# carlosmwh1985/BspAtom

Hardware: AMD Instinct MI355X
Metric: l-channel eigensolves/sec at N_bsp=4096 fp64 (higher is better)
Workload: dtype f64; 1 GPU; Hydrogen Coulomb l=0..127, N_bsp=4096, k=9, KIND_GRID=0 rb=800 (BASELINE configs[3]); `value` = weak scaling: 128 l-channels per GPU, 128 in total; channels_total=128, eigenvector_owner_rank=0, collective_calls=0, launched_by=python

## Files before the change

bspatom_amd/csrc/capi.hip:

```cpp
#include <atomic>
#include <new>
#include "capi_internal.h"

using namespace bsp;

namespace bsp {
static std::atomic<int> g_process_device{-1};
int process_device() { return g_process_device.load(); }
int process_device_check(int device)
{
    const int cur = g_process_device.load();
    if (cur >= 0 && cur != device) {
        fprintf(stderr, "bspatom: this process already works on device %d; use one process per GPU (device %d refused)\n", cur, device);
        return BSP_ERR_UNSUPPORTED;
    }
    return BSP_OK;
}
void process_device_latch(int device) { int expect = -1; g_process_device.compare_exchange_strong(expect, device); }

int device_cus()
{
    static const int cus = [] {
        int dev = 0, v = 0;
        return (hipGetDevice(&dev) == hipSuccess && hipDeviceGetAttribute(&v, hipDeviceAttributeMultiprocessorCount, dev) == hipSuccess && v > 0) ? v : 256;
    }();
    return cus;
}

hipError_t LaunchCtx::sync()
{
    hipError_t first = hipSuccess;
    auto wait = [&](hipStream_t s) {
        const hipError_t e = s ? hipStreamSynchronize(s) : hipSuccess;
        if (first == hipSuccess) first = e;
    };
    for (hipStream_t s : cw_aux) wait(s);
    for (const Sy2sbLane &ln : lanes) { wait(ln.main); wait(ln.side); }
    return first;
}

void LaunchCtx::release()
{
    (void)sync();
    auto drop_stream = [](hipStream_t &s) { if (s) (void)hipStreamDestroy(s); s = nullptr; };
    auto drop_event = [](hipEvent_t &e) { if (e) (void)hipEventDestroy(e); e = nullptr; };
    for (hipStream_t &s : cw_aux) drop_stream(s);
    drop_event(cw_fork);
    for (hipEvent_t &e : cw_join) drop_event(e);
    for (Sy2sbLane &ln : lanes) { drop_stream(ln.main); drop_stream(ln.side); drop_event(ln.evA); drop_event(ln.evB); drop_event(ln.done); }
    drop_event(sy_fork);
    (void)hipFree(bis_tail); (void)hipFree(bis_qcnt); (void)hipFree(sb2st_chk);
    bis_tail = nullptr; bis_tail_cap = 0; bis_qcnt = nullptr; sb2st_chk = nullptr;
}
}

namespace {
struct OptName { const char *name; const char *env; int Options::*field; };
const OptName OPT_TABLE[] = {
    {"sb2st_version", "BSP_SB2ST_VERSION", &Options::sb2st_version},
    {"sb2st_ring", "BSP_SB2ST_RING", &Options::sb2st_ring},
    {"sb2st_margin", "BSP_SB2ST_MARGIN", &Options::sb2st_margin},
    {"sb2st_hyst", "BSP_SB2ST_HYST", &Options::sb2st_hyst},
    {"sb2st_lead", "BSP_SB2ST_LEAD", &Options::sb2st_lead},
    {"sb2st_check", "BSP_SB2ST_CHECK", &Options::sb2st_check},
    {"sb2st_diag", "BSP_SB2ST_DIAG", &Options::sb2st_diag},
    {"sb2st_force_abort", "BSP_SB2ST_FORCE_ABORT", &Options::sb2st_force_abort},
    {"sy2sb_groups", "BSP_SY2SB_GROUPS", &Options::sy2sb_groups},
    {"sy2sb_lookahead", "BSP_SY2SB_LOOKAHEAD", &Options::sy2sb_lookahead},
    {"sy2sb_segs", "BSP_SY2SB_SEGS", &Options::sy2sb_segs},
    {"panel_qr", "BSP_PANEL_QR", &Options::panel_qr},
    {"gemm_diag", "BSP_GEMM_DIAG", &Options::gemm_diag},
    {"bisect", "BSP_BISECT", &Options::bisect},
    {"bisect_ept", "BSP_BISECT_EPT", &Options::bisect_ept},
    {"bisect_tail", "BSP_BISECT_TAIL", &Options::bisect_tail},
    {"bisect_secant", "BSP_BISECT_SECANT", &Options::bisect_secant},
    {"bisect_pair", "BSP_BISECT_PAIR", &Options::bisect_pair},
    {"bisect_queue", "BSP_BISECT_QUEUE", &Options::bisect_queue},
    {"bisect_queue_grid", "BSP_BISECT_QUEUE_GRID", &Options::bisect_queue_grid},
    {"bisect_diag", "BSP_BISECT_DIAG", &Options::bisect_diag},
    {"no_eigvec_prefetch", "BSP_NO_EIGVEC_PREFETCH", &Options::no_eigvec_prefetch},
    {"vec_early", "BSP_VEC_EARLY", &Options::vec_early},
    {"vec_own_cu", "BSP_VEC_OWN_CU", &Options::vec_own_cu},
    {"poison_c", "BSP_POISON_C", &Options::poison_c},
    {"sb2sb_mfma", "BSP_SB2SB_MFMA", &Options::sb2sb_mfma},
    {"ktime", "BSP_KTIME", &Options::ktime},
    {"tsqr_regcap", "BSP_TSQR_REGCAP", &Options::tsqr_regcap},
    {"tsqr_max_m", "BSP_TSQR_MAX_M", &Options::tsqr_max_m},
    {"sb16_rows", "BSP_SB16_ROWS", &Options::sb16_rows},
    {"route", "BSP_ROUTE", &Options::route},
    {"cw_onediv", "BSP_CW_ONEDIV", &Options::cw_onediv},
    {"cw_items4", "BSP_CW_ITEMS4", &Options::cw_items4},
    {"cw_bcast", "BSP_CW_BCAST", &Options::cw_bcast},
    {"cw_nw", "BSP_CW_NW", &Options::cw_nw},
    {"cw_ldspad", "BSP_CW_LDSPAD", &Options::cw_ldspad},
    {"cw_ipw", "BSP_CW_IPW", &Options::cw_ipw},
    {"cw_band8", "BSP_CW_BAND8", &Options::cw_band8},
    {"cw_split", "BSP_CW_SPLIT", &Options::cw_split},
    {"cw_diag", "BSP_CW_DIAG", &Options::cw_diag},
    {"s_overlap", "BSP_S_OVERLAP", &Options::s_overlap},
    {"cw_streams", "BSP_CW_STREAMS", &Options::cw_streams},
    {"cw_chunk_min", "BSP_CW_CHUNK_MIN", &Options::cw_chunk_min},
    {"sb8_wgs", "BSP_SB8_WGS", &Options::sb8_wgs},
    {"sbr_phased", "BSP_SBR_PHASED", &Options::sbr_phased},
    {"sbr_lag", "BSP_SBR_LAG", &Options::sbr_lag},
    {"fused_probe", "BSP_FUSED_PROBE", &Options::fused_probe},
    {"dipole_stage_mb", "BSP_DIPOLE_STAGE_MB", &Options::dipole_stage_mb},
    {"resolvent_stage_mb", "BSP_RESOLVENT_STAGE_MB", &Options::resolvent_stage_mb},
    {"resolvent_slots", "BSP_RESOLVENT_SLOTS", &Options::resolvent_slots},
    {"wf_stage_mb", "BSP_WF_STAGE_MB", &Options::wf_stage_mb},
    {"tdse_stage_mb", "BSP_TDSE_STAGE_MB", &Options::tdse_stage_mb},
    {"tdse_adapt_group", "BSP_TDSE_ADAPT_GROUP", &Options::tdse_adapt_group},
    {"tdse_spline_group", "BSP_TDSE_SPLINE_GROUP", &Options::tdse_spline_group},
};
}

namespace bsp {
Options &opts()
{
    static Options o = [] {
        Options v;
        for (const OptName &t : OPT_TABLE) {
            const char *e = getenv(t.env);
            if (e) v.*(t.field) = (*e == 0) ? 1 : atoi(e);
        }
        return v;
    }();
    return o;
}

namespace {
struct KRec { int slot; hipEvent_t e0, e1; };
std::vector<KRec> g_krecs;
std::vector<hipEvent_t> g_kpool;
hipEvent_t g_kopen[KS_COUNT];
hipEvent_t kevent()
{
    hipEvent_t e = nullptr;
    if (!g_kpool.empty()) { e = g_kpool.back(); g_kpool.pop_back(); }
    else if (hipEventCreate(&e) != hipSuccess) e = nullptr;
    return e;
}
const char *const KSLOT_NAMES[KS_COUNT] = {"gemm2_kernel<128,128,MODE 1> (rank-128 update, syr2k)", "gemm2_kernel<64,128,MODE 2> (symm Y = A22 W)",
                                          "panel_qr2_kernel / panel_qr_kernel", "sy2sb chain: G, K (split-K gemm_kernel + splitk_reduce), form_T, tsmm64 (W, Z)",
                                          "sb2sb_mfma_kernel (band 64 -> 16)", "sbr_rows_kernel<8> / <16> / sb16st_kernel (one-column chase to tridiagonal)", "bisect3_kernel",
                                          "band_cholesky_kernel + std_form_kernel",
                                          "crawford_item_kernel and its set-up kernels (band route: pencil -> band 15)",
                                          "operator_band_kernel (bands of caller-given g(r), g(r) d/dr)",
                                          "tdse_stage_kernel (one Runge-Kutta stage of bspatom_tdse_propagate)"};
}
void ktime_begin(int slot, hipStream_t st)
{
    hipEvent_t e = kevent();
    g_kopen[slot] = e;
    if (e) (void)hipEventRecord(e, st);
}
void ktime_end(int slot, hipStream_t st)
{
    hipEvent_t e0 = g_kopen[slot], e1 = kevent();
    g_kopen[slot] = nullptr;
    if (!e0 || !e1) return;
    (void)hipEventRecord(e1, st);
    g_krecs.push_back({slot, e0, e1});
}
}

extern "C" int bspatom_kernel_times(double *ms, int32_t *launches, int cap)
{
    if (!ms || !launches || cap < KS_COUNT) return BSP_ERR_ARG;
    BSP_HIP(hipDeviceSynchronize());
    for (int i = 0; i < cap; ++i) { ms[i] = 0.0; launches[i] = 0; }
    for (const auto &r : g_krecs) {
        float t = 0.f;
        if (hipEventElapsedTime(&t, r.e0, r.e1) == hipSuccess) { ms[r.slot] += t; launches[r.slot] += 1; }
        g_kpool.push_back(r.e0); g_kpool.push_back(r.e1);
    }
    g_krecs.clear();
    return KS_COUNT;
}

extern "C" const char *bspatom_kernel_slot_name(int slot)
{
    return (slot >= 0 && slot < KS_COUNT) ? KSLOT_NAMES[slot] : nullptr;
}

extern "C" int bspatom_set_option(const char *name, int value)
{
    if (!name) return BSP_ERR_ARG;
    for (const OptName &t : OPT_TABLE)
        if (!strcmp(name, t.name)) { opts().*(t.field) = value; return BSP_OK; }
    return BSP_ERR_ARG;
}

extern "C" int bspatom_get_option(const char *name, int *value)
{
    if (!name || !value) return BSP_ERR_ARG;
    for (const OptName &t : OPT_TABLE)
        if (!strcmp(name, t.name)) { *value = opts().*(t.field); return BSP_OK; }
    return BSP_ERR_ARG;
}

extern "C" void bspatom_input_defaults(bspatom_input *in) { input_defaults(in); }

extern "C" int bspatom_device_count(void)
{
    int n = 0;
    if (hipGetDeviceCount(&n) != hipSuccess) return 0;
    return n;
}

static int derive_checked(const bspatom_input &in, HostSetup *h)
{
    const int drc = derive(in, h);
    if (drc == -5) {
        fprintf(stderr, "bspatom: B-spline order k = %d (Gauss-Legendre points ka = %d) exceeds the limits k <= %d, ka <= %d of this build\n",
                in.k, h->ka, BSPATOM_MAX_K, BSPATOM_MAX_KA);
        return BSP_ERR_UNSUPPORTED;
    }
    return drc ? BSP_ERR_ARG : BSP_OK;
}

static void fill_sizes(const HostSetup &h, int npad, bspatom_sizes *s)
{
    s->nfun = h.nfun; s->k = h.k; s->ka = h.ka; s->nkp = h.nkp; s->nointv = h.nointv;
    s->nbc1 = h.nbc1; s->nbc2 = h.nbc2; s->lmax = h.lmax; s->nintv_exp = h.nintv_exp;
    s->nintv_lin = h.nintv_lin; s->npad = npad;
}

static void copy_grid(const HostSetup &h, double *rt, double *aind, double *xg, double *wg)
{
    if (rt) memcpy(rt, h.rt.data(), h.rt.size() * sizeof(double));
    if (aind) memcpy(aind, h.aind.data(), h.aind.size() * sizeof(double));
    if (xg) memcpy(xg, h.xg.data(), h.xg.size() * sizeof(double));
    if (wg) memcpy(wg, h.wg.data(), h.wg.size() * sizeof(double));
}

extern "C" int bspatom_host_setup(const bspatom_input *in, bspatom_sizes *s, double *rt, double *aind, double *xg,
                                  double *wg)
{
    if (!in || !s) return BSP_ERR_ARG;
    HostSetup h;
    int rc;
    if ((rc = derive_checked(*in, &h))) return rc;
    fill_sizes(h, round_up(h.nfun, 64), s);
    if (rt || aind || xg || wg) {
        build_grid(&h);
        copy_grid(h, rt, aind, xg, wg);
    }
    return BSP_OK;
}

static void free_solve_buffers(bspatom_problem *p)
{
    hipFree(p->d_SB); hipFree(p->d_HB); hipFree(p->d_UB); hipFree(p->d_rdiag); hipFree(p->d_Y);
    hipFree(p->d_C); hipFree(p->d_AB); hipFree(p->d_d); hipFree(p->d_e); hipFree(p->d_E); hipFree(p->d_work); hipFree(p->d_sbctl);
    hipFree(p->d_cwork);
    p->d_SB = p->d_HB = p->d_UB = p->d_rdiag = p->d_Y = p->d_C = p->d_AB = p->d_d = p->d_e = p->d_E = nullptr;
    p->d_work = nullptr; p->d_sbctl = nullptr; p->d_cwork = nullptr;
    p->cap_nl = 0; p->cap_dense = 0; p->cap_band = 0;
}

extern "C" void bspatom_problem_destroy(bspatom_problem *p)
{
    if (!p) return;
    hipSetDevice(p->device);
    if (p->st) (void)hipStreamSynchronize(p->st);
    p->lc.release();
    free_solve_buffers(p);
    hipFree(p->d_rt); hipFree(p->d_aind); hipFree(p->d_xg); hipFree(p->d_wg); hipFree(p->d_vpot);
    hipFree(p->d_bl); hipFree(p->d_ptab); hipFree(p->d_left); hipFree(p->d_status); hipFree(p->d_info);
    hipFree(p->d_vwork); hipFree(p->d_vec); hipFree(p->d_wfr); hipFree(p->d_wfu); hipFree(p->d_Esel); hipFree(p->d_chan);
    hipFree(p->d_pvec); hipFree(p->d_pE); hipFree(p->d_pinfo);
    if (p->st2) hipStreamDestroy(p->st2);
    if (p->evx) hipEventDestroy(p->evx);
    if (p->stS) hipStreamDestroy(p->stS);
    if (p->evS) hipEventDestroy(p->evS);
    for (hipEvent_t e : p->evC) if (e) hipEventDestroy(e);
    for (auto &e : p->ev) if (e) hipEventDestroy(e);
    if (p->st) hipStreamDestroy(p->st);
    delete p;
}

template <class T>
static int upload(T **dst, const T *src, size_t count)
{
    BSP_HIP(hipMalloc(reinterpret_cast<void **>(dst), count * sizeof(T)));
    BSP_HIP(hipMemcpy(*dst, src, count * sizeof(T), hipMemcpyHostToDevice));
    return BSP_OK;
}

static int problem_init(bspatom_problem *p, const bspatom_input *in, int device)
{
    int rc;
    if ((rc = derive_checked(*in, &p->hs))) return rc;
    if (p->hs.nfun > BSPATOM_MAX_NFUN) {
        fprintf(stderr, "bspatom: nfun = %d exceeds the %d functions per channel this build supports\n", p->hs.nfun, BSPATOM_MAX_NFUN);
        return BSP_ERR_UNSUPPORTED;
    }
    build_grid(&p->hs);
    build_vpot(&p->hs);
    p->device = device;
    p->npad = round_up(p->hs.nfun, 64);
    BSP_HIP(hipSetDevice(device));
    BSP_HIP(hipStreamCreate(&p->st));
    for (auto &e : p->ev) BSP_HIP(hipEventCreate(&e));
    const HostSetup &h = p->hs;
    if ((rc = upload(&p->d_rt, h.rt.data(), h.rt.size())) || (rc = upload(&p->d_aind, h.aind.data(), h.aind.size())) ||
        (rc = upload(&p->d_xg, h.xg.data(), h.xg.size())) || (rc = upload(&p->d_wg, h.wg.data(), h.wg.size())) ||
        (rc = upload(&p->d_vpot, h.vpot.data(), h.vpot.size())) || (rc = upload(&p->d_bl, h.bl, (size_t)4))) return rc;
    const size_t npt = (size_t)(h.nkp - 1) * h.ka;
    BSP_HIP(hipMalloc(reinterpret_cast<void **>(&p->d_ptab), npt * (2 * h.k + 3) * sizeof(double)));
    BSP_HIP(hipMalloc(reinterpret_cast<void **>(&p->d_left), npt * sizeof(int)));
    BSP_HIP(hipMalloc(reinterpret_cast<void **>(&p->d_status), sizeof(int)));
    BSP_HIP(hipMemset(p->d_status, 0, sizeof(int)));
    return BSP_OK;
}

extern "C" int bspatom_problem_create(const bspatom_input *in, int device, bspatom_problem **out)
{
    if (!in || !out) return BSP_ERR_ARG;
    *out = nullptr;
    int ndev = 0;
    if (hipGetDeviceCount(&ndev) != hipSuccess || ndev <= 0 || device < 0 || device >= ndev) {
        fprintf(stderr, "bspatom: no HIP device %d (libbspatom has no CPU path)\n", device);
        return BSP_ERR_NOGPU;
    }
    int rc0;
    if ((rc0 = bsp::process_device_check(device))) return rc0;
    bspatom_problem *p = new (std::nothrow) bspatom_problem;
    if (!p) return BSP_ERR_ARG;
    p->device = device;
    const int rc = problem_init(p, in, device);
    if (rc) { bspatom_problem_destroy(p); return rc; }
    bsp::process_device_latch(device);
    *out = p;
    return BSP_OK;
}

extern "C" int bspatom_problem_sizes(const bspatom_problem *p, bspatom_sizes *s)
{
    if (!p || !s) return BSP_ERR_ARG;
    fill_sizes(p->hs, p->npad, s);
    return BSP_OK;
}

extern "C" int bspatom_problem_route(const bspatom_problem *p)
{
    if (!p) return BSP_ERR_ARG;
    return pipeline_route(p->hs.nfun, p->hs.k);
}

extern "C" int bspatom_problem_grid(const bspatom_problem *p, double *rt, double *aind, double *xg, double *wg)
{
    if (!p) return BSP_ERR_ARG;
    copy_grid(p->hs, rt, aind, xg, wg);
    return BSP_OK;
}

static int ensure_capacity(bspatom_problem *p, int nl)
{
    if (nl <= p->cap_nl) return BSP_OK;
    free_solve_buffers(p);
    p->last_nl = 0; p->pre_l = -1;
    p->band_nl = 0;
    const HostSetup &h = p->hs;
    const size_t n = h.nfun, k = h.k, np = p->npad, b = nl;
    BSP_HIP(hipMalloc(reinterpret_cast<void **>(&p->d_SB), k * n * sizeof(double)));
    BSP_HIP(hipMalloc(reinterpret_cast<void **>(&p->d_HB), b * k * n * sizeof(double)));
    BSP_HIP(hipMalloc(reinterpret_cast<void **>(&p->d_UB), k * n * sizeof(double)));
    BSP_HIP(hipMalloc(reinterpret_cast<void **>(&p->d_rdiag), n * sizeof(double)));
    BSP_HIP(hipMalloc(reinterpret_cast<void **>(&p->d_AB), b * ab_stride((int)np) * sizeof(double)));
    BSP_HIP(hipMalloc(reinterpret_cast<void **>(&p->d_d), b * np * sizeof(double)));
    BSP_HIP(hipMalloc(reinterpret_cast<void **>(&p->d_e), b * np * sizeof(double)));
    BSP_HIP(hipMalloc(reinterpret_cast<void **>(&p->d_E), b * n * sizeof(double)));
    BSP_HIP(hipMalloc(&p->d_sbctl, sb2st_ctl_bytes(nl)));
    if (!p->d_info) BSP_HIP(hipMalloc(reinterpret_cast<void **>(&p->d_info), sizeof(int)));
    p->cap_nl = nl;
    return BSP_OK;
}

static int ensure_route_buffers(bspatom_problem *p, int nl, int route)
{
    const HostSetup &h = p->hs;
    const size_t np = p->npad, b = nl;
    if (route == 2 && nl > p->cap_band) {
        hipFree(p->d_cwork); p->d_cwork = nullptr; p->cap_band = 0;
        BSP_HIP(hipMalloc(&p->d_cwork, crawford_work_bytes(h.nfun, h.k, nl)));
        p->cap_band = nl;
    }
    if (route == 1 && nl > p->cap_dense) {
        hipFree(p->d_Y); hipFree(p->d_C); hipFree(p->d_work);
        p->d_Y = p->d_C = nullptr; p->d_work = nullptr; p->cap_dense = 0;
        BSP_HIP(hipMalloc(reinterpret_cast<void **>(&p->d_Y), b * np * np * sizeof(double)));
        BSP_HIP(hipMalloc(reinterpret_cast<void **>(&p->d_C), b * np * np * sizeof(double)));
        BSP_HIP(hipMalloc(&p->d_work, sy2sb_work_bytes((int)np, 64, nl)));
        p->cap_dense = nl;
    }
    return BSP_OK;
}

static int enqueue_assemble(bspatom_problem *p, int l0, int nl, int skip = 0, double *sb_other = nullptr)
{
    const HostSetup &h = p->hs;
    int rc;
    if ((rc = ensure_point_table(p))) return rc;
    if (nl - skip <= 0) return BSP_OK;
    return launch_assemble_bands(h.nfun, h.k, h.ka, h.nkp, h.in.kind_pot, p->d_bl, l0 + skip, nl - skip, p->d_ptab, p->d_left,
                                 skip ? sb_other : p->d_SB, p->d_HB + (size_t)skip * h.k * h.nfun, p->st);
}

extern "C" int bspatom_assemble(bspatom_problem *p, int l0, int nl, double *SB, double *HB)
{
    if (!p || nl <= 0 || l0 < 0) return BSP_ERR_ARG;
    BSP_HIP(hipSetDevice(p->device));
    int rc;
    if ((rc = ensure_capacity(p, nl))) return rc;
    p->last_nl = 0; p->pre_l = -1;
    p->band_nl = 0;
    if ((rc = enqueue_assemble(p, l0, nl))) return rc;
    BSP_HIP(hipStreamSynchronize(p->st));
    if ((rc = check_status(p))) return rc;
    p->band_l0 = l0; p->band_nl = nl;
    const size_t kn = (size_t)p->hs.k * p->hs.nfun;
    if (SB) BSP_HIP(hipMemcpy(SB, p->d_SB, kn * sizeof(double), hipMemcpyDeviceToHost));
    if (HB) BSP_HIP(hipMemcpy(HB, p->d_HB, kn * nl * sizeof(double), hipMemcpyDeviceToHost));
    return BSP_OK;
}

namespace bsp {
int pipeline_route(int n, int k)
{
    const int r = opts().route;
    if (r == 1) return 1;
    if (r == 2) return 2;
    return (crawford_supported(n, k) && n >= 32) ? 2 : 1;
}

int pipeline_enqueue(LaunchCtx &cx, int n, int npad, int k, int nl, const double *d_SB, const double *d_HB, const PipeBufs &b,
                     double *d_Eout, hipStream_t st, hipEvent_t *ev, bool with_bisect, bool s_prepared)
{
    int rc;
    const int route = pipeline_route(n, k);
    if (route == 2) {
        if (!crawford_supported(n, k)) {
            fprintf(stderr, "bspatom: BSP_ROUTE=2 (band route) takes pencils of half-width k - 1 <= 8 and n >= 16 (k = %d, n = %d)\n", k, n);
            return BSP_ERR_UNSUPPORTED;
        }
        if (!b.cwork) return BSP_ERR_ARG;
        CrawfordWork cw;
        crawford_carve(b.cwork, n, k, nl, &cw);
        if (ev) BSP_HIP(hipEventRecord(ev[1], st));
        if ((rc = crawford_run(cx, n, npad, k, nl, d_SB, d_HB, cw, b.AB, st, s_prepared, b.s_events))) return rc;
        if (ev) BSP_HIP(hipEventRecord(ev[2], st));
        if (b.chase_after) BSP_HIP(hipStreamWaitEvent(st, b.chase_after, 0));
        if ((rc = launch_sb16st(n, npad, nl, b.AB, b.d, b.e, st, b.status, b.sbctl, opts().cw_band8 ? 8 : 16))) return rc;
        if (ev) BSP_HIP(hipEventRecord(ev[3], st));
        if (!with_bisect) return BSP_OK;
        if ((rc = launch_bisect(cx, n, npad, nl, b.d, b.e, d_Eout, n, st))) return rc;
        if (ev) BSP_HIP(hipEventRecord(ev[4], st));
        return BSP_OK;
    }
    if (!b.Y || !b.C || !b.work) return BSP_ERR_ARG;
    if (opts().poison_c) BSP_HIP(hipMemsetAsync(b.C, 0xFF, (size_t)nl * npad * npad * sizeof(double), st));
    {
        KScope kt(KS_STDFORM, st);
        if ((rc = launch_band_cholesky(n, k, d_SB, b.UB, b.rdiag, b.info, st))) return rc;
        if ((rc = launch_standard_form(n, npad, k, nl, d_HB, b.UB, b.rdiag, b.Y, b.C, st))) return rc;
    }
    if (ev) BSP_HIP(hipEventRecord(ev[1], st));
    Sy2sbWork w;
    sy2sb_carve(b.work, npad, 64, nl, &w);
    if ((rc = sy2sb_run(cx, npad, 64, nl, b.C, w, st))) return rc;
    if ((rc = launch_extract_band(npad, 64, nl, b.C, b.AB, st))) return rc;
    if (ev) BSP_HIP(hipEventRecord(ev[2], st));
    if ((rc = launch_sb2st(cx, n, npad, 64, nl, b.AB, b.d, b.e, st, b.status, b.sbctl))) return rc;
    if (ev) BSP_HIP(hipEventRecord(ev[3], st));
    if (!with_bisect) return BSP_OK;
    if ((rc = launch_bisect(cx, n, npad, nl, b.d, b.e, d_Eout, n, st))) return rc;
    if (ev) BSP_HIP(hipEventRecord(ev[4], st));
    return BSP_OK;
}
}

int bsp::ensure_vec_scratch(bspatom_problem *p)
{
    const HostSetup &h = p->hs;
    if (p->d_vwork) return BSP_OK;
    BSP_HIP(hipMalloc(reinterpret_cast<void **>(&p->d_vwork), invit_work_doubles(h.nfun, h.k) * sizeof(double)));
    BSP_HIP(hipMalloc(reinterpret_cast<void **>(&p->d_vec), (size_t)h.nfun * sizeof(double)));
    BSP_HIP(hipMalloc(reinterpret_cast<void **>(&p->d_chan), sizeof(int)));
    BSP_HIP(hipMalloc(reinterpret_cast<void **>(&p->d_Esel), sizeof(double)));
    return BSP_OK;
}

static int solve_enqueue(bspatom_problem *p, int l0, int nl, int route, double *E_dev_out)
{
    const HostSetup &h = p->hs;
    const int n = h.nfun, np = p->npad;
    int rc;
    BSP_HIP(hipMemsetAsync(p->d_info, 0, sizeof(int), p->st));
    BSP_HIP(hipEventRecord(p->ev[0], p->st));
    bool s_prepared = false;
    if (route == 2 && nl > 1 && opts().s_overlap) {
        if (!p->stS) {
            BSP_HIP(hipStreamCreateWithFlags(&p->stS, hipStreamNonBlocking));
            BSP_HIP(hipEventCreateWithFlags(&p->evS, hipEventDisableTiming));
            for (hipEvent_t &e : p->evC) BSP_HIP(hipEventCreateWithFlags(&e, hipEventDisableTiming));
        }
        if ((rc = enqueue_assemble(p, l0, 1))) return rc;
        BSP_HIP(hipEventRecord(p->evS, p->st));
        BSP_HIP(hipStreamWaitEvent(p->stS, p->evS, 0));
        CrawfordWork cw;
        crawford_carve(p->d_cwork, n, h.k, nl, &cw);
        if ((rc = crawford_prepare(n, h.k, p->d_SB, cw, p->stS, p->evC))) return rc;
        if ((rc = enqueue_assemble(p, l0, nl, 1, p->d_UB))) return rc;
        s_prepared = true;
    } else if ((rc = enqueue_assemble(p, l0, nl))) return rc;
    BSP_HIP(hipEventRecord(p->ev[1], p->st));
    p->pre_l = -1; p->pre_early = false;
    const int tl = h.in.l_ini, tn0 = h.in.n0_ini;
    const bool want_vec = tl >= l0 && tl < l0 + nl && tn0 >= 1 && tn0 <= n && !opts().no_eigvec_prefetch;
    const bool early = want_vec && route == 2 && opts().vec_early;
    auto side_stream = [&]() -> int {
        if (!p->st2) {
            BSP_HIP(hipStreamCreateWithFlags(&p->st2, hipStreamNonBlocking));
            BSP_HIP(hipEventCreateWithFlags(&p->evx, hipEventDisableTiming));
            BSP_HIP(hipMalloc(reinterpret_cast<void **>(&p->d_pvec), (size_t)n * sizeof(double)));
            BSP_HIP(hipMalloc(reinterpret_cast<void **>(&p->d_pE), sizeof(double)));
            BSP_HIP(hipMalloc(reinterpret_cast<void **>(&p->d_pinfo), sizeof(int)));
        }
        return ensure_vec_scratch(p);
    };
    if (early) {
        if ((rc = side_stream())) return rc;
        p->pre_ch = tl - l0;
        hipStream_t sv = s_prepared ? p->stS : p->st2;
        const int cus = device_cus();
        const bool own_cu = opts().vec_own_cu == 2 || (opts().vec_own_cu == 1 && ((nl + 7) / 8) * 8 * 8 > cus);
        BSP_HIP(hipMemsetAsync(p->d_pinfo, 0, sizeof(int), sv));
        if (s_prepared && tl == l0) BSP_HIP(hipStreamWaitEvent(sv, p->evS, 0));
        else {
            BSP_HIP(hipEventRecord(p->evx, p->st));
            BSP_HIP(hipStreamWaitEvent(sv, p->evx, 0));
        }
        if ((rc = launch_early_vector(n, h.k, p->d_SB, p->d_HB + (size_t)p->pre_ch * h.k * n, tn0 - 1, p->d_pE, p->d_vwork, p->d_pvec,
                                      p->d_pinfo, sv, own_cu))) return rc;
        BSP_HIP(hipEventRecord(p->evx, sv));
        p->pre_l = tl; p->pre_n0 = tn0; p->pre_early = true;
    }
    PipeBufs pb{p->d_UB, p->d_rdiag, p->d_Y, p->d_C, p->d_AB, p->d_d, p->d_e, p->d_work, p->d_info, p->d_status, p->d_sbctl, p->d_cwork, s_prepared ? p->evC : nullptr,
                (early && opts().vec_early == 3) ? p->evx : nullptr};
    double *Eout = E_dev_out ? E_dev_out : p->d_E;
    if ((rc = pipeline_enqueue(p->lc, n, np, h.k, nl, p->d_SB, p->d_HB, pb, Eout, p->st, &p->ev[1], false, s_prepared))) return rc;
    if (want_vec && !early) {
        if ((rc = side_stream())) return rc;
        p->pre_ch = tl - l0;
        const int ch = p->pre_ch;
        BSP_HIP(hipMemcpyAsync(p->d_chan, &p->pre_ch, sizeof(int), hipMemcpyHostToDevice, p->st));
        BSP_HIP(hipMemsetAsync(p->d_pinfo, 0, sizeof(int), p->st));
        rc = launch_bisect_one(n, p->d_d + (size_t)ch * np, p->d_e + (size_t)ch * np, tn0 - 1, p->d_pE, p->st);
        if (rc == BSP_ERR_UNSUPPORTED) rc = BSP_OK;
        else if (rc) return rc;
        else {
            BSP_HIP(hipEventRecord(p->evx, p->st));
            BSP_HIP(hipStreamWaitEvent(p->st2, p->evx, 0));
            if ((rc = launch_inverse_iteration(n, h.k, 1, p->d_SB, p->d_HB, p->d_chan, p->d_pE, p->d_vwork, p->d_pvec,
                                               p->d_pinfo, p->st2))) return rc;
            BSP_HIP(hipEventRecord(p->evx, p->st2));
            p->pre_l = tl; p->pre_n0 = tn0;
        }
    }
    if ((rc = launch_bisect(p->lc, n, np, nl, p->d_d, p->d_e, Eout, n, p->st))) return rc;
    BSP_HIP(hipEventRecord(p->ev[5], p->st));
    if (p->pre_l >= 0) BSP_HIP(hipStreamWaitEvent(p->st, p->evx, 0));
    if (E_dev_out)
        BSP_HIP(hipMemcpyAsync(p->d_E, E_dev_out, (size_t)nl * n * sizeof(double), hipMemcpyDeviceToDevice, p->st));
    BSP_HIP(hipStreamSynchronize(p->st));
    return BSP_OK;
}

static int solve_collect(bspatom_problem *p, int l0, int nl, int route, double *E_host, int32_t *info)
{
    const HostSetup &h = p->hs;
    const int n = h.nfun, tn0 = h.in.n0_ini;
    int rc;
    for (int i = 0; i < 5; ++i) {
        float ms = 0.f;
        hipEventElapsedTime(&ms, p->ev[i], p->ev[i + 1]);
        p->ms[i] = ms;
    }
    float tot = 0.f;
    hipEventElapsedTime(&tot, p->ev[0], p->ev[5]);
    p->ms[5] = tot;
    if ((rc = check_status(p))) return rc;
    if (p->pre_early) {
        const int m = tn0 - 1, i0 = m > 0 ? m - 1 : 0, i1 = m < n - 1 ? m + 1 : n - 1;
        double ev[3] = {0, 0, 0}, lb = 0, ends[2];
        const double *Erow = p->d_E + (size_t)p->pre_ch * n;
        BSP_HIP(hipMemcpy(ev, Erow + i0, (size_t)(i1 - i0 + 1) * sizeof(double), hipMemcpyDeviceToHost));
        BSP_HIP(hipMemcpy(&ends[0], Erow, sizeof(double), hipMemcpyDeviceToHost));
        BSP_HIP(hipMemcpy(&ends[1], Erow + n - 1, sizeof(double), hipMemcpyDeviceToHost));
        BSP_HIP(hipMemcpy(&lb, p->d_pE, sizeof(double), hipMemcpyDeviceToHost));
        const double width = fmax(fabs(ends[0]), fabs(ends[1])), em = ev[m - i0], dist = fabs(lb - em);
        bool ok = dist <= 1e-10 * width;
        for (int i = i0; i <= i1; ++i)
            if (i != m && fabs(lb - ev[i - i0]) < dist) ok = false;
        if (!ok || opts().vec_early == 2) p->pre_l = -1;
        p->pre_early_ok = ok;
    }
    int cinfo = 0;
    if (route == 2) {
        CrawfordWork cw;
        crawford_carve(p->d_cwork, n, h.k, nl, &cw);
        BSP_HIP(hipMemcpy(&cinfo, cw.info, sizeof(int), hipMemcpyDeviceToHost));
        if (cinfo) {
            if ((rc = launch_band_cholesky(n, h.k, p->d_SB, p->d_UB, p->d_rdiag, p->d_info, p->st))) return rc;
            BSP_HIP(hipStreamSynchronize(p->st));
            BSP_HIP(hipMemcpy(&cinfo, p->d_info, sizeof(int), hipMemcpyDeviceToHost));
            if (!cinfo) cinfo = 1;
        }
    } else
    BSP_HIP(hipMemcpy(&cinfo, p->d_info, sizeof(int), hipMemcpyDeviceToHost));
    if (info)
        for (int l = 0; l < nl; ++l) info[l] = cinfo ? n + cinfo : 0;
    if (E_host) BSP_HIP(hipMemcpy(E_host, p->d_E, (size_t)nl * n * sizeof(double), hipMemcpyDeviceToHost));
    p->last_l0 = l0; p->last_nl = nl;
    p->band_l0 = l0; p->band_nl = nl;
    return BSP_OK;
}

static int solve_impl(bspatom_problem *p, int l0, int nl, double *E_dev_out, double *E_host, int32_t *info)
{
    if (!p || nl <= 0 || l0 < 0) return BSP_ERR_ARG;
    BSP_HIP(hipSetDevice(p->device));
    int rc;
    if ((rc = ensure_capacity(p, nl))) return rc;
    const int route = pipeline_route(p->hs.nfun, p->hs.k);
    if ((rc = ensure_route_buffers(p, nl, route))) return rc;
    p->last_nl = 0; p->band_nl = 0;
    if (!(rc = solve_enqueue(p, l0, nl, route, E_dev_out))) rc = solve_collect(p, l0, nl, route, E_host, info);
    if (rc) {
        (void)hipStreamSynchronize(p->st);
        if (p->st2) (void)hipStreamSynchronize(p->st2);
        if (p->stS) (void)hipStreamSynchronize(p->stS);
        (void)p->lc.sync();
    }
    return rc;
}

extern "C" int bspatom_solve(bspatom_problem *p, int l0, int nl, double *E, int32_t *info)
{
    return solve_impl(p, l0, nl, nullptr, E, info);
}

extern "C" int bspatom_solve_dev(bspatom_problem *p, int l0, int nl, double *E_dev, int32_t *info)
{
    if (!E_dev) return BSP_ERR_ARG;
    return solve_impl(p, l0, nl, E_dev, nullptr, info);
}

extern "C" int bspatom_early_vector_state(const bspatom_problem *p, int32_t *state)
{
    if (!p || !state) return BSP_ERR_ARG;
    *state = !p->pre_early ? 0 : (p->pre_early_ok ? 1 : -1);
    return BSP_OK;
}

extern "C" int bspatom_last_timing(const bspatom_problem *p, double ms[6])
{
    if (!p || !ms) return BSP_ERR_ARG;
    for (int i = 0; i < 6; ++i) ms[i] = p->ms[i];
    return BSP_OK;
}
```

bspatom_amd/csrc/common.h:

```cpp
#pragma once
#include <hip/hip_runtime.h>
#include <cstdint>
#include <cstdio>
#include <cstdlib>

#define BSP_OK 0
#define BSP_ERR_HIP (-1)
#define BSP_ERR_ARG (-2)
#define BSP_ERR_BSPLVB (-3)
#define BSP_ERR_NOGPU (-4)
#define BSP_ERR_UNSUPPORTED (-5)

#define BSP_HIP(x)                                                                          \
    do {                                                                                    \
        hipError_t e_ = (x);                                                                \
        if (e_ != hipSuccess) {                                                             \
            fprintf(stderr, "bspatom: HIP error '%s' at %s:%d\n", hipGetErrorString(e_),    \
                    __FILE__, __LINE__);                                                    \
            return BSP_ERR_HIP;                                                             \
        }                                                                                   \
    } while (0)

typedef double double4_t __attribute__((ext_vector_type(4)));

__host__ __device__ inline size_t ab_stride(int npad) { return (size_t)npad * 128 + 1088; }

namespace bsp {

struct Options {
    int sb2st_version = 0;
    int sb2st_ring = 0;
    int sb2st_margin = 3, sb2st_hyst = 2;
    int sb2st_lead = 0;
    int sb2st_check = 0;
    int sb2st_diag = 0;
    int sb2st_force_abort = 0;
    int sy2sb_groups = 2, sy2sb_lookahead = 1, sy2sb_segs = 0;
    int panel_qr = 3;
    int tsqr_max_m = 2048;
    int tsqr_regcap = 1;
    int gemm_diag = 0;
    int bisect = 3, bisect_ept = 0;
    int bisect_secant = 1;
    int bisect_tail = 1;
    int bisect_pair = 1;
    int bisect_queue = 1;
    int bisect_queue_grid = 0;
    int bisect_diag = 0;
    int no_eigvec_prefetch = 0;
    int vec_early = 1;
    int vec_own_cu = 1;
    int sb2sb_mfma = 1;
    int sb16_rows = 1;
    int poison_c = 0;
    int route = 0;
    int fused_probe = 0;
    int cw_items4 = 1;
    int cw_nw = 1;
    int cw_streams = 2;
    int cw_chunk_min = 1024;
    int s_overlap = 1;
    int cw_diag = 0;
    int cw_split = 0;
    int cw_band8 = 1;
    int sb8_wgs = 0;
    int sbr_phased = 1;
    int sbr_lag = 0;
    int cw_ipw = 0;
    int cw_ldspad = 0;
    int cw_onediv = 0;
    int cw_bcast = 1;
    int dipole_stage_mb = 0;
    int wf_stage_mb = 0;
    int tdse_stage_mb = 0;
    int tdse_adapt_group = 0;
    int tdse_spline_group = 0;
    int resolvent_stage_mb = 0;
    int resolvent_slots = 0;
    int ktime = 0;
};
Options &opts();

int process_device();
int process_device_check(int device);
void process_device_latch(int device);
int device_cus();

template <class K>
inline hipError_t allow_lds(K kernel, size_t bytes)
{
    return hipFuncSetAttribute(reinterpret_cast<const void *>(kernel), hipFuncAttributeMaxDynamicSharedMemorySize, (int)bytes);
}
template <class K>
inline int persistent_slots(K kernel, int threads, size_t lds_bytes, int items, int *slots)
{
    int per_cu = 0;
    const int cus = device_cus();
    BSP_HIP(hipOccupancyMaxActiveBlocksPerMultiprocessor(&per_cu, kernel, threads, lds_bytes));
    const long r = (long)(per_cu > 0 ? per_cu : 1) * (cus > 0 ? cus : 1);
    *slots = (int)(r < items ? r : items);
    return BSP_OK;
}

struct Sy2sbLane {
    hipStream_t main = nullptr, side = nullptr;
    hipEvent_t evA = nullptr, evB = nullptr, done = nullptr;
};
constexpr int SY2SB_MAXG = 4;
struct LaunchCtx {
    hipStream_t cw_aux[3] = {nullptr, nullptr, nullptr};
    hipEvent_t cw_fork = nullptr, cw_join[3] = {nullptr, nullptr, nullptr};
    Sy2sbLane lanes[SY2SB_MAXG];
    hipEvent_t sy_fork = nullptr;
    double2 *bis_tail = nullptr;
    size_t bis_tail_cap = 0;
    unsigned *bis_qcnt = nullptr;
    int *sb2st_chk = nullptr;

    LaunchCtx() = default;
    LaunchCtx(const LaunchCtx &) = delete;
    LaunchCtx &operator=(const LaunchCtx &) = delete;
    ~LaunchCtx() { release(); }
    hipError_t sync();
    void release();
};

enum KSlot { KS_SYR2K = 0, KS_SYMM, KS_PANEL_QR, KS_CHAIN, KS_SB2SB, KS_SB16ST, KS_BISECT, KS_STDFORM, KS_CRAWFORD, KS_OPBAND, KS_TDSE, KS_COUNT };
void ktime_begin(int slot, hipStream_t st);
void ktime_end(int slot, hipStream_t st);
struct KScope {
    int slot; hipStream_t st; bool on;
    KScope(int slot_, hipStream_t st_) : slot(slot_), st(st_), on(opts().ktime != 0) { if (on) ktime_begin(slot, st); }
    ~KScope() { if (on) ktime_end(slot, st); }
};

struct GemmDesc {
    int M, N, K, batch;
    const double *A; long sAm, sAk, bA;
    const double *B; long sBk, sBn, bB;
    double *C; long sCm, sCn, bC;
    double alpha, beta;
    int lower_only;
    int yoff;
    int ksplit;
    int kchunk;
    long bCs;
    int nsb, toff;
    int sbpre[80];
    int sbxy[80];
};
int gemm_f64(const GemmDesc &g, hipStream_t st);
int gemm_splitk_f64(const GemmDesc &g, int splits, double *part, hipStream_t st);
int tsmm64_f64(int m, int batch, const double *A, long lda, long bsA, const double *B, long bsB, double *C, long ldc, long bsC,
               double alpha, double beta, hipStream_t st);
int syr2k_lower_f64(int m, int batch, double *A22, long ld, long bsA, const double *buf, long ldb, long bsBuf, int seg, int nseg,
                    int part, hipStream_t st);
int symm_lower_f64(int m, int batch, const double *A22, long ld, long bsA, const double *W, long ldw, long bsW,
                   double *Y, long ldy, long bsY, hipStream_t st);

int launch_point_table(int nkp, int k, int ka, int nfun, const double *d_rt, const double *d_aind,
                       const double *d_xg, const double *d_wg, const double *d_vpot, double *d_ptab,
                       int *d_left, int *d_status, hipStream_t st);
int launch_assemble_bands(int nfun, int k, int ka, int nkp, int kind_pot, const double *d_bl, int l0,
                          int nl, const double *d_ptab, const int *d_left, double *d_SB, double *d_HB,
                          hipStream_t st);
int launch_dipole_bands(int nfun, int k, int ka, int nkp, const double *d_ptab, const int *d_left, double *d_RB,
                        hipStream_t st);
int launch_band_cholesky(int n, int k, const double *d_SB, double *d_UB, double *d_rdiag, int *d_info,
                         hipStream_t st);
int launch_band_cholesky_range(int n, int k, int jstart, int jstop, const double *d_SB, double *d_UB, double *d_rdiag, int *d_info,
                               hipStream_t st);
int launch_band_cholesky_pair(int n, int k, int jstop, const double *d_SB, double *d_UB, double *d_rdiag, int *d_info, hipStream_t st);
int launch_standard_form(int n, int npad, int k, int nl, const double *d_HB, const double *d_UB,
                         const double *d_rdiag, double *d_Y, double *d_C, hipStream_t st, int full = 0);
struct CrawfordWork {
    double *SBf, *UBf, *rdiagf;
    double *Qel, *LiB;
    double *D, *E, *G;
    double *U;
    int *info;
};
bool crawford_supported(int n, int k);
size_t crawford_work_bytes(int n, int k, int nl);
void crawford_carve(void *base, int n, int k, int nl, CrawfordWork *w);
constexpr int CW_CHUNKS = 4;
int crawford_prepare(int n, int k, const double *d_SB, const CrawfordWork &w, hipStream_t st, hipEvent_t *evc = nullptr);
int crawford_run(LaunchCtx &cx, int n, int npad, int k, int nl, const double *d_SB, const double *d_HB, const CrawfordWork &w, double *d_AB,
                 hipStream_t st, bool s_prepared = false, hipEvent_t *evc = nullptr);
long tsqr_scr_doubles(int npad);
long tsqr_cntr_ints(int npad);
int tsqr_panel(int npad, int r0, int c0, int batch, double *d_A, double *buf, double *W, double *scr, int *cntr, hipStream_t st);
struct Sy2sbWork {
    double *tsqr_scr;
    int *tsqr_cntr;
    double *buf2;
    double *tau2;
    double *buf;
    double *W;
    double *G;
    double *T;
    double *Kmat;
    double *tau;
    double *part;
};
constexpr int SY2SB_SPLITK = 16;
size_t sy2sb_work_bytes(int npad, int nb, int batch);
void sy2sb_carve(void *base, int npad, int nb, int batch, Sy2sbWork *w);
int sy2sb_run(LaunchCtx &cx, int npad, int nb, int batch, double *d_A, const Sy2sbWork &w, hipStream_t st);
int sy2sb_panel_only(int npad, int c0, int batch, double *d_A, const Sy2sbWork &w, hipStream_t st);
int launch_extract_band(int npad, int nb, int batch, const double *d_A, double *d_AB, hipStream_t st);
size_t sb2st_ctl_bytes(int batch);
int launch_sb2sb(int n, int npad, int batch, double *d_AB, hipStream_t st);
int launch_sb16st(int n, int npad, int batch, double *d_AB, double *d_d, double *d_e, hipStream_t st, int *d_status, void *ctl, int hb = 16);
int launch_sb2st(LaunchCtx &cx, int n, int npad, int b, int batch, double *d_AB, double *d_d, double *d_e, hipStream_t st, int *d_status,
                 void *ctl);
int launch_bisect(LaunchCtx &cx, int n, int ldn, int batch, const double *d_d, const double *d_e, double *d_w, long ldw, hipStream_t st);
int launch_bisect_one(int n, const double *d_d, const double *d_e, int m, double *d_out, hipStream_t st);
int launch_band_multisect(int n, int k, const double *d_SB, const double *d_HB, int m, double *d_out, hipStream_t st);
constexpr size_t OWN_CU_LDS = 144 * 1024;
int launch_early_vector(int n, int k, const double *d_SB, const double *d_HB, int m, double *d_E, double *d_work, double *d_vec,
                        int *d_info, hipStream_t st, bool own_cu);
int launch_inverse_iteration(int n, int k, int nvec, const double *d_SB, const double *d_HB,
                             const int *d_chan, const double *d_E, double *d_work, double *d_vec,
                             int *d_info, hipStream_t st, const int *d_start = nullptr, int rank = 0);
size_t invit_work_doubles(int n, int k);
size_t invit_batch_slot_doubles(int n, int k);
int invit_batch_slots(int k, int items, int *slots);
int launch_inverse_iteration_batch(int n, int k, int count, int items, int slots, const double *d_SB, const double *d_HB,
                                   const double *d_E, double *d_work, double *d_vec, int *d_info, hipStream_t st);
int launch_band_apply(int n, int k, const double *d_RB, const double a[3], const double *d_x, double *d_v, hipStream_t st);
int launch_dots(int n, int m, const double *d_Z, const double *d_v, double *d_D, hipStream_t st);
int launch_band_apply_block(int n, int k, int count, int nitems, const double *d_RB, const double *d_acoef, const long long *d_xoff,
                            const double *d_base, double *d_W, hipStream_t st);
void dipole_kslices(int n, int count_ini, int count_fin, int *chunk, int *nslices);
int launch_dipole_block(int n, int count_ini, int count_fin, int npairs, const long long *d_pw, const double *d_base, double *d_part,
                        double *d_out, hipStream_t st);
int launch_operator_bands(int nfun, int k, int ka, int nkp, int nop, int nr, const double *d_ptab, const int *d_left,
                          const int *d_qfirst, const double *d_g, const int *d_deriv, double *d_GB, hipStream_t st);
int launch_band_combine_apply(int n, int k, int nop, int count, int nitems, const double *d_GB, const double *d_acoef,
                              const long long *d_xoff, const double *d_base, double *d_W, hipStream_t st);
struct ResolventArgs {
    int n, k, nmat, nrhs, nproj;
    const double *SB, *HB;
    const int *chan;
    const double *z, *WB;
    const int *w;
    const double *B, *P;
    double *X, *R;
    int *info;
    double *work;
};
size_t resolvent_slot_doubles(int n, int k);
int resolvent_slots(int k, int nmat, int *slots);
int launch_resolvent(const ResolventArgs &a, int slots, hipStream_t st);
struct ResolventChainArgs {
    int n, k, nchain, nstage, nop, nrhs, nproj;
    const double *SB, *HB;
    const int *chan;
    const double *z, *WB;
    const int *w;
    const double *GB, *acoef;
    const double *B, *P;
    double *X, *R;
    int *info;
    double *work;
};
size_t resolvent_chain_slot_doubles(int n, int k, int nrhs);
int resolvent_chain_slots(int k, int nchain, int *slots);
int launch_resolvent_chain(const ResolventChainArgs &a, int slots, hipStream_t st);
struct ResolventCoupledArgs {
    int n, k, nch, nmat, nrhs, nproj, ncoup, nop;
    const double *SB, *HB;
    const int *chan;
    const double *z, *WB;
    const int *w;
    const int *cr, *cc, *ctr;
    const double *GB, *acoef;
    const double *B, *P;
    double *X, *R;
    int *info;
    double *work;
};
int resolvent_coupled_max_band();
size_t resolvent_coupled_slot_doubles(int n, int k, int nch);
int resolvent_coupled_slots(int k, int nch, int nmat, int *slots);
int launch_resolvent_coupled(const ResolventCoupledArgs &a, int slots, hipStream_t st);
int resolvent_wide_max_band();
size_t resolvent_wide_slot_doubles(int n, int k, int nch, int nrhs);
int resolvent_wide_slots(int k, int nch, int nmat, int *slots);
int launch_resolvent_wide(const ResolventCoupledArgs &a, int slots, hipStream_t st);
struct TdseSplineArgs {
    ResolventCoupledArgs m;
    int nscan, n0, nst, snap_every, s0, obs_every, j0, fin, jfin;
    double g;
    double *c, *snap, *obs;
};
int tdse_spline_slots(int k, int nch, int nscan, int *slots);
int launch_tdse_spline(const TdseSplineArgs &a, int slots, hipStream_t st);
int tdse_spline_wide_slots(int k, int nch, int nscan, int *slots);
int launch_tdse_spline_wide(const TdseSplineArgs &a, int slots, hipStream_t st);
int launch_wf_tabulate(int nkp, int k, int n, const double *d_rt, const double *d_c, double ra,
                       double rb, int npts, double *d_r, double *d_u, int *d_status, hipStream_t st);
int wf_quadrature(int nkp, int ka, const double *rt, const double *xg, const double *wg, int *rows, double *r, double *w);
bool wf_points_valid(int nkp, const double *rt, int npts, const double *r);
int launch_basis_table(int nkp, int k, int nfun, int npts, const double *d_rt, const double *d_aind, const double *d_r, double *d_tab,
                       int *d_tleft, int *d_status, hipStream_t st);
int launch_basis_gather(int k, int npts, const int *d_rows, const double *d_ptab, const int *d_pleft, double *d_tab, int *d_tleft,
                        hipStream_t st);
int launch_tabulate(int k, int nfun, int npts, int nvec, const double *d_tab, const int *d_tleft, const double *d_Z, double *d_U,
                    double *d_dU, hipStream_t st);
struct TdseDims { int nch, count, nscan, NC; };
struct TdseBufs {
    const int *cptr, *ent;
    const double *E, *D;
    double *a, *K;
    unsigned long long *err2;
    double *part;
    const double *ph;
    const double *W = nullptr;
    int ow = 4;
    int nf = 1;
};
int tdse_columns(int nscan);
int launch_tdse_step(const TdseDims &d, const TdseBufs &w, const double *d_field, double dt, double *d_snap, double *d_obs, hipStream_t st);
int launch_tdse_observe(const TdseDims &d, const TdseBufs &w, const double *d_field, double *d_row, hipStream_t st);
int launch_tdse_phases(const TdseDims &d, const double *d_E, double dt, double *d_ph, hipStream_t st);
int launch_tdse_pack(const TdseDims &d, const double *d_user, double *d_work, hipStream_t st);
int launch_tdse_unpack(const TdseDims &d, const double *d_work, double *d_user, hipStream_t st);

struct TdseAdaptCtl {
    int n, m, j;
    int flag;
    int done;
    int nend;
    int row, snap;
    int row0, snap0, node0;
    int pad_;
    long long acc_t;
    long long stats[6];
};
constexpr size_t TDSE_CTL_HDR = 128;
static_assert(sizeof(TdseAdaptCtl) <= TDSE_CTL_HDR, "the arrays of the control block start behind its header");
inline size_t tdse_ctl_bytes(int nscan) { return TDSE_CTL_HDR + (size_t)13 * nscan * sizeof(double); }
__host__ __device__ inline const double *tdse_ctl_fld(const TdseAdaptCtl *c) { return (const double *)((const char *)c + TDSE_CTL_HDR); }
struct TdseAdaptArgs {
    int nsub, max_level, snap_every, obs_every, log_cap;
    double dt, tol;
    const double *fn;
    int *log_i;
    double *log_e, *log_f;
};
int launch_tdse_adapt_init(const TdseDims &d, const TdseBufs &w, TdseAdaptCtl *ctl, const TdseAdaptArgs &g, hipStream_t st);
int launch_tdse_adapt_attempt(const TdseDims &d, const TdseBufs &w, TdseAdaptCtl *ctl, const TdseAdaptArgs &g, long long t, double *cand,
                              size_t phlev, double *d_snap, double *d_obs, hipStream_t st);

struct PipeBufs {
    double *UB, *rdiag, *Y, *C, *AB, *d, *e;
    void *work;
    int *info;
    int *status = nullptr;
    void *sbctl = nullptr;
    void *cwork = nullptr;
    hipEvent_t *s_events = nullptr;
    hipEvent_t chase_after = nullptr;
};
int pipeline_route(int n, int k);
size_t pipe_bytes_per_channel(int npad);
int pipeline_enqueue(LaunchCtx &cx, int n, int npad, int k, int nl, const double *d_SB, const double *d_HB,
                     const PipeBufs &b, double *d_Eout, hipStream_t st, hipEvent_t *ev, bool with_bisect = true, bool s_prepared = false);

}
```

bspatom_amd/csrc/sbr2.hip:

```cpp
#include "common.h"
#include "wave_ops.h"
#include <cstdio>
#include <cstdlib>

namespace bsp {
namespace {

constexpr int LD = 128;
constexpr int B1 = 64, NB1 = 16, LAG = 3;
constexpr int XLD = 65, VLD = 17;
constexpr int SB2SB_LDS = (64 * XLD + 3 * 64 * VLD + 16 * XLD + 2 * 16 * VLD + 16) * 8;

__device__ __forceinline__ double wsum64(double v)
{
    for (int m = 32; m; m >>= 1) v += __shfl_xor(v, m);
    return v;
}

__global__ __launch_bounds__(256) void sb2sb_kernel(int n, int npad, double *__restrict__ ABall, int t, int s_lo)
{
    extern __shared__ double lds[];
    double *X = lds, *V = X + 64 * XLD, *Y = V + 64 * VLD, *Z = Y + 64 * VLD, *W = Z + 64 * VLD, *T = W + 16 * XLD,
           *G = T + 16 * VLD, *tau = G + 16 * VLD;
    const int tid = threadIdx.x, lane = tid & 63, wv = tid >> 6;
    const int s = s_lo + blockIdx.x, k = t - LAG * s;
    if (k < 0) return;
    const int j0 = NB1 * s, r0 = j0 + NB1 + B1 * k;
    if (r0 >= n) return;
    double *AB = ABall + blockIdx.y * ab_stride(npad);
    const int pc0 = k == 0 ? j0 : r0 - B1;
    const int ncl = k == 0 ? NB1 : B1;
    const int gi = r0 + lane;

    for (int c = wv; c < ncl; c += 4) {
        const int gc = pc0 + c;
        X[c * XLD + lane] = gi < n ? AB[(size_t)gc * LD + (gi - gc)] : 0.0;
    }
    __syncthreads();
    for (int i = 0; i < NB1; ++i) {
        if (wv == 0) {
            const double x = X[i * XLD + lane];
            const double nrm2 = wsum64(lane > i ? x * x : 0.0);
            const double alpha = X[i * XLD + i];
            double tq = 0.0, scale = 0.0, beta = alpha;
            if (nrm2 != 0.0) {
                beta = -copysign(sqrt(alpha * alpha + nrm2), alpha);
                tq = (beta - alpha) / beta;
                scale = 1.0 / (alpha - beta);
            }
            V[lane * VLD + i] = lane < i ? 0.0 : (lane == i ? 1.0 : x * scale);
            if (lane == 0) tau[i] = tq;
            X[i * XLD + lane] = lane < i ? x : (lane == i ? beta : 0.0);
        }
        __syncthreads();
        const double tq = tau[i];
        for (int j = i + 1 + wv; j < NB1; j += 4) {
            const double v = V[lane * VLD + i], x = X[j * XLD + lane];
            const double dot = wsum64(v * x);
            X[j * XLD + lane] = x - tq * dot * v;
        }
        __syncthreads();
    }
    {
        const int i = tid >> 4, j = tid & 15;
        double a = 0.0;
        for (int r = 0; r < 64; ++r) a += V[r * VLD + i] * V[r * VLD + j];
        G[i * VLD + j] = a;
        T[i * VLD + j] = 0.0;
    }
    __syncthreads();
    for (int i = 0; i < NB1; ++i) {
        if (tid < i) {
            double a = 0.0;
            for (int m = tid; m < i; ++m) a += T[tid * VLD + m] * G[m * VLD + i];
            T[tid * VLD + i] = -tau[i] * a;
        }
        if (tid == i) T[i * VLD + i] = tau[i];
        __syncthreads();
    }
    if (k > 0) {
        const int i = tid & 15, c = 16 + (tid >> 4) * 3;
        double a0 = 0.0, a1 = 0.0, a2 = 0.0;
        for (int r = 0; r < 64; ++r) {
            const double v = V[r * VLD + i];
            a0 += v * X[c * XLD + r]; a1 += v * X[(c + 1) * XLD + r]; a2 += v * X[(c + 2) * XLD + r];
        }
        W[i * XLD + c] = a0; W[i * XLD + c + 1] = a1; W[i * XLD + c + 2] = a2;
        __syncthreads();
        double b0 = 0.0, b1 = 0.0, b2 = 0.0;
        for (int j = 0; j <= i; ++j) {
            const double tj = T[j * VLD + i];
            b0 += tj * W[j * XLD + c]; b1 += tj * W[j * XLD + c + 1]; b2 += tj * W[j * XLD + c + 2];
        }
        __syncthreads();
        W[i * XLD + c] = b0; W[i * XLD + c + 1] = b1; W[i * XLD + c + 2] = b2;
        __syncthreads();
        double vr[16];
        for (int q = 0; q < 16; ++q) vr[q] = V[lane * VLD + q];
        for (int cc = 16 + wv * 12; cc < 16 + wv * 12 + 12; ++cc) {
            double a = X[cc * XLD + lane];
            for (int q = 0; q < 16; ++q) a -= vr[q] * W[q * XLD + cc];
            X[cc * XLD + lane] = a;
        }
        __syncthreads();
    }
    for (int c = wv; c < ncl; c += 4) {
        const int gc = pc0 + c;
        if (gi < n) AB[(size_t)gc * LD + (gi - gc)] = X[c * XLD + lane];
    }
    __syncthreads();

    for (int c = wv; c < 64; c += 4) {
        if (lane >= c) {
            const double v = gi < n ? AB[(size_t)(r0 + c) * LD + (lane - c)] : 0.0;
            X[c * XLD + lane] = v;
            X[lane * XLD + c] = v;
        }
    }
    __syncthreads();
    {
        double y0 = 0.0, y1 = 0.0, y2 = 0.0, y3 = 0.0;
        for (int c = 0; c < 64; ++c) {
            const double d = X[c * XLD + lane];
            const double *vc = V + c * VLD + 4 * wv;
            y0 += d * vc[0]; y1 += d * vc[1]; y2 += d * vc[2]; y3 += d * vc[3];
        }
        double *yr = Y + lane * VLD + 4 * wv;
        yr[0] = y0; yr[1] = y1; yr[2] = y2; yr[3] = y3;
    }
    __syncthreads();
    for (int q = 0; q < 4; ++q) {
        const int i = 4 * wv + q;
        double a = 0.0;
        for (int m = 0; m <= i; ++m) a += Y[lane * VLD + m] * T[m * VLD + i];
        Z[lane * VLD + i] = a;
    }
    __syncthreads();
    {
        const int i = tid >> 4, j = tid & 15;
        double a = 0.0;
        for (int r = 0; r < 64; ++r) a += V[r * VLD + i] * Z[r * VLD + j];
        G[i * VLD + j] = a;
    }
    __syncthreads();
    {
        const int i = tid >> 4, j = tid & 15;
        double a = 0.0;
        for (int m = 0; m <= i; ++m) a += T[m * VLD + i] * G[m * VLD + j];
        W[i * XLD + j] = a;
    }
    __syncthreads();
    for (int q = 0; q < 4; ++q) {
        const int i = 4 * wv + q;
        double a = 0.0;
        for (int m = 0; m < 16; ++m) a += V[lane * VLD + m] * W[m * XLD + i];
        Z[lane * VLD + i] -= 0.5 * a;
    }
    __syncthreads();
    {
        double vr[16], zr[16];
        for (int q = 0; q < 16; ++q) { vr[q] = V[lane * VLD + q]; zr[q] = Z[lane * VLD + q]; }
        for (int c = 16 * wv; c < 16 * wv + 16; ++c) {
            if (lane >= c) {
                double a = X[c * XLD + lane];
                for (int q = 0; q < 16; ++q) a -= vr[q] * Z[c * VLD + q] + zr[q] * V[c * VLD + q];
                if (gi < n) AB[(size_t)(r0 + c) * LD + (lane - c)] = a;
            }
        }
    }
    __syncthreads();

    const int r1 = r0 + B1;
    if (r1 >= n) return;
    const int gi1 = r1 + lane;
    for (int c = wv; c < 64; c += 4) {
        const int gc = r0 + c;
        X[c * XLD + lane] = gi1 < n ? AB[(size_t)gc * LD + (gi1 - gc)] : 0.0;
    }
    __syncthreads();
    {
        double y0 = 0.0, y1 = 0.0, y2 = 0.0, y3 = 0.0;
        for (int c = 0; c < 64; ++c) {
            const double d = X[c * XLD + lane];
            const double *vc = V + c * VLD + 4 * wv;
            y0 += d * vc[0]; y1 += d * vc[1]; y2 += d * vc[2]; y3 += d * vc[3];
        }
        double *yr = Y + lane * VLD + 4 * wv;
        yr[0] = y0; yr[1] = y1; yr[2] = y2; yr[3] = y3;
    }
    __syncthreads();
    for (int q = 0; q < 4; ++q) {
        const int i = 4 * wv + q;
        double a = 0.0;
        for (int m = 0; m <= i; ++m) a += Y[lane * VLD + m] * T[m * VLD + i];
        Z[lane * VLD + i] = a;
    }
    __syncthreads();
    {
        double zr[16];
        for (int q = 0; q < 16; ++q) zr[q] = Z[lane * VLD + q];
        for (int c = 16 * wv; c < 16 * wv + 16; ++c) {
            double a = X[c * XLD + lane];
            for (int q = 0; q < 16; ++q) a -= zr[q] * V[c * VLD + q];
            if (gi1 < n) AB[(size_t)(r0 + c) * LD + (gi1 - (r0 + c))] = a;
        }
    }
}

typedef double d4_t __attribute__((ext_vector_type(4)));
constexpr int SB2SB2_LDS = (64 * XLD + 4 * 64 * VLD + 16 * VLD + 16) * 8;

#define MFMA(a, b, c) __builtin_amdgcn_mfma_f64_16x16x4f64((a), (b), (c), 0, 0, 0)

__global__ __launch_bounds__(256) void sb2sb_mfma_kernel(int n, int npad, double *__restrict__ ABall, int t, int s_lo)
{
    extern __shared__ double lds[];
    double *X = lds, *V = X + 64 * XLD, *VT = V + 64 * VLD, *Yb = VT + 64 * VLD, *Z = Yb + 64 * VLD, *G = Z + 64 * VLD,
           *tau = G + 16 * VLD;
    double *Gp = Z;
    const int tid = threadIdx.x, lane = tid & 63, w = tid >> 6, l15 = lane & 15, l4 = lane >> 4;
    const int s = s_lo + blockIdx.x, k = t - LAG * s;
    if (k < 0) return;
    const int j0 = NB1 * s, r0 = j0 + NB1 + B1 * k;
    if (r0 >= n) return;
    double *AB = ABall + blockIdx.y * ab_stride(npad);
    const int pc0 = k == 0 ? j0 : r0 - B1;
    const int ncl = k == 0 ? NB1 : B1;
    const int gi = r0 + lane;

    const bool rin = gi < n;
    const int gr = rin ? gi : r0;
    double xc[4], lt[12], pf[16];
    for (int q = 0; q < 4; ++q) {
        const int gc = pc0 + w + 4 * q;
        xc[q] = AB[(size_t)gc * LD + (gr - gc)];
    }
    if (k > 0) {
#pragma unroll
        for (int q = 0; q < 12; ++q) {
            const int gc = pc0 + 16 + w + 4 * q;
            lt[q] = AB[(size_t)gc * LD + (gr - gc)];
        }
    }
#pragma unroll
    for (int q = 0; q < 16; ++q) {
        const int c = w + 4 * q;
        const bool in = lane >= c && rin;
        pf[q] = AB[in ? (size_t)(r0 + c) * LD + (lane - c) : 0];
    }
    for (int q = 0; q < 4; ++q) xc[q] = rin ? xc[q] : 0.0;
    auto make_reflector = [&](const int i) {
        const double x = xc[i >> 2];
        const double nrm2 = wave_sum(lane > i ? x * x : 0.0);
        const double alpha = read_lane(x, i);
        double tq = 0.0, scale = 0.0, beta = alpha;
        if (nrm2 != 0.0) {
            beta = -copysign(sqrt(alpha * alpha + nrm2), alpha);
            tq = (beta - alpha) / beta;
            scale = 1.0 / (alpha - beta);
        }
        V[lane * VLD + i] = lane < i ? 0.0 : (lane == i ? 1.0 : x * scale);
        if (lane == 0) tau[i] = tq;
        xc[i >> 2] = lane < i ? x : (lane == i ? beta : 0.0);
    };
    if (w == 0) make_reflector(0);
    lds_barrier();
#pragma unroll
    for (int i = 0; i < NB1 - 1; ++i) {
        const double v = V[lane * VLD + i], tq = tau[i];
        if (w == ((i + 1) & 3)) {
            const int q1 = (i + 1) >> 2;
            const double dot = wave_sum(v * xc[q1]);
            xc[q1] -= tq * dot * v;
            make_reflector(i + 1);
        }
#pragma unroll
        for (int q = 0; q < 4; ++q)
            if (w + 4 * q > i + 1) {
                const double dot = wave_sum(v * xc[q]);
                xc[q] -= tq * dot * v;
            }
        lds_barrier();
    }
    for (int q = 0; q < 4; ++q) {
        const int gc = pc0 + w + 4 * q;
        if (gi < n) AB[(size_t)gc * LD + (gi - gc)] = xc[q];
    }
    if (k > 0) {
#pragma unroll
        for (int q = 0; q < 12; ++q) X[(16 + w + 4 * q) * XLD + lane] = rin ? lt[q] : 0.0;
    }
    {
        d4_t acc = {0.0, 0.0, 0.0, 0.0};
        for (int q = 0; q < 4; ++q) {
            const double a = V[(16 * w + 4 * q + l4) * VLD + l15];
            acc = MFMA(a, a, acc);
        }
        for (int r = 0; r < 4; ++r) Gp[w * 16 * VLD + (l4 + 4 * r) * VLD + l15] = acc[r];
    }
    lds_barrier();
    {
        const int i = tid >> 4, j = tid & 15, o = i * VLD + j;
        G[o] = (Gp[o] + Gp[16 * VLD + o]) + (Gp[32 * VLD + o] + Gp[48 * VLD + o]);
    }
    lds_barrier();
    if (w == 0) {
        double vt[16];
#pragma unroll
        for (int j = 0; j < 16; ++j) {
            double a = V[lane * VLD + j];
#pragma unroll
            for (int i = 0; i < j; ++i) a -= vt[i] * G[i * VLD + j];
            vt[j] = a * tau[j];
            VT[lane * VLD + j] = vt[j];
        }
    }
    lds_barrier();

    if (k > 0) {
        if (w < 3) {
            d4_t acc = {0.0, 0.0, 0.0, 0.0};
            const int cn = 16 + 16 * w + l15;
            for (int q = 0; q < 16; ++q) acc = MFMA(VT[(4 * q + l4) * VLD + l15], X[cn * XLD + 4 * q + l4], acc);
            for (int r = 0; r < 4; ++r) Yb[(l4 + 4 * r) * XLD + cn] = acc[r];
        }
        lds_barrier();
        for (int nb = 0; nb < 3; ++nb) {
            const int cn = 16 + 16 * nb + l15;
            d4_t acc;
            for (int r = 0; r < 4; ++r) acc[r] = X[cn * XLD + 16 * w + l4 + 4 * r];
            for (int q = 0; q < 4; ++q) acc = MFMA(-V[(16 * w + l15) * VLD + 4 * q + l4], Yb[(4 * q + l4) * XLD + cn], acc);
            for (int r = 0; r < 4; ++r) X[cn * XLD + 16 * w + l4 + 4 * r] = acc[r];
        }
        lds_barrier();
        for (int c = 16 + w; c < 64; c += 4) {
            const int gc = pc0 + c;
            if (gi < n) AB[(size_t)gc * LD + (gi - gc)] = X[c * XLD + lane];
        }
        lds_barrier();
    }

#pragma unroll
    for (int q = 0; q < 16; ++q) {
        const int c = w + 4 * q;
        if (lane >= c) {
            const double v = gi < n ? pf[q] : 0.0;
            X[c * XLD + lane] = v;
            X[lane * XLD + c] = v;
        }
    }
    const int r1 = r0 + B1, gi1 = r1 + lane;
    const bool more = r1 < n;
    if (more) {
#pragma unroll
        for (int q = 0; q < 16; ++q) {
            const int gc = r0 + w + 4 * q;
            pf[q] = AB[gi1 < n ? (size_t)gc * LD + (gi1 - gc) : 0];
        }
    }
    lds_barrier();
    {
        d4_t acc = {0.0, 0.0, 0.0, 0.0};
        for (int q = 0; q < 16; ++q) acc = MFMA(X[(4 * q + l4) * XLD + 16 * w + l15], VT[(4 * q + l4) * VLD + l15], acc);
        for (int r = 0; r < 4; ++r) Yb[(16 * w + l4 + 4 * r) * VLD + l15] = acc[r];
    }
    lds_barrier();
    {
        d4_t acc = {0.0, 0.0, 0.0, 0.0};
        for (int q = 4 * w; q < 4 * w + 4; ++q) acc = MFMA(VT[(4 * q + l4) * VLD + l15], Yb[(4 * q + l4) * VLD + l15], acc);
        for (int r = 0; r < 4; ++r) Gp[w * 16 * VLD + (l4 + 4 * r) * VLD + l15] = acc[r];
    }
    lds_barrier();
    {
        const int i = tid >> 4, j = tid & 15, o = i * VLD + j;
        G[o] = (Gp[o] + Gp[16 * VLD + o]) + (Gp[32 * VLD + o] + Gp[48 * VLD + o]);
    }
    lds_barrier();
    {
        d4_t acc;
        for (int r = 0; r < 4; ++r) acc[r] = Yb[(16 * w + l4 + 4 * r) * VLD + l15];
        for (int q = 0; q < 4; ++q) acc = MFMA(-0.5 * V[(16 * w + l15) * VLD + 4 * q + l4], G[(4 * q + l4) * VLD + l15], acc);
        for (int r = 0; r < 4; ++r) Z[(16 * w + l4 + 4 * r) * VLD + l15] = acc[r];
    }
    lds_barrier();
    for (int bi = w; bi < 10; bi += 4) {
        const int mb = bi < 1 ? 0 : (bi < 3 ? 1 : (bi < 6 ? 2 : 3));
        const int nb = bi - (mb * (mb + 1)) / 2;
        d4_t acc;
        for (int r = 0; r < 4; ++r) acc[r] = X[(16 * nb + l15) * XLD + 16 * mb + l4 + 4 * r];
        for (int q = 0; q < 4; ++q) {
            acc = MFMA(-V[(16 * mb + l15) * VLD + 4 * q + l4], Z[(16 * nb + l15) * VLD + 4 * q + l4], acc);
            acc = MFMA(-Z[(16 * mb + l15) * VLD + 4 * q + l4], V[(16 * nb + l15) * VLD + 4 * q + l4], acc);
        }
        for (int r = 0; r < 4; ++r) X[(16 * nb + l15) * XLD + 16 * mb + l4 + 4 * r] = acc[r];
    }
    lds_barrier();
    for (int c = w; c < 64; c += 4)
        if (lane >= c && gi < n) AB[(size_t)(r0 + c) * LD + (lane - c)] = X[c * XLD + lane];

    if (!more) return;
    lds_barrier();
#pragma unroll
    for (int q = 0; q < 16; ++q) X[(w + 4 * q) * XLD + lane] = gi1 < n ? pf[q] : 0.0;
    lds_barrier();
    {
        d4_t acc = {0.0, 0.0, 0.0, 0.0};
        for (int q = 0; q < 16; ++q) acc = MFMA(X[(4 * q + l4) * XLD + 16 * w + l15], VT[(4 * q + l4) * VLD + l15], acc);
        for (int r = 0; r < 4; ++r) Yb[(16 * w + l4 + 4 * r) * VLD + l15] = acc[r];
    }
    lds_barrier();
    for (int nb = 0; nb < 4; ++nb) {
        d4_t acc;
        for (int r = 0; r < 4; ++r) acc[r] = X[(16 * nb + l15) * XLD + 16 * w + l4 + 4 * r];
        for (int q = 0; q < 4; ++q) acc = MFMA(-Yb[(16 * w + l15) * VLD + 4 * q + l4], V[(16 * nb + l15) * VLD + 4 * q + l4], acc);
        for (int r = 0; r < 4; ++r) X[(16 * nb + l15) * XLD + 16 * w + l4 + 4 * r] = acc[r];
    }
    lds_barrier();
    for (int c = w; c < 64; c += 4) {
        const int gc = r0 + c;
        if (gi1 < n) AB[(size_t)gc * LD + (gi1 - gc)] = X[c * XLD + lane];
    }
}
#undef MFMA

constexpr int B2 = 16, NW2 = 8, WCOLS = 512, WROWS = 32;
constexpr int SB16_LDS = (WCOLS * WROWS + NW2 * 16 + 2) * 8;


__device__ __forceinline__ void house_params(double alpha, double nrm2, double &beta, double &tq, double &scale)
{
    beta = -copysign(sqrt(alpha * alpha + nrm2), alpha);
    tq = (beta - alpha) / beta;
    scale = 1.0 / (alpha - beta);
}

template <bool FAST>
__device__ __forceinline__ void chase_item(double *Lw, double *pS, int r0, int c0, int k, int r, int g, int cA, int cT,
                                           const int (&offD)[4])
{
#define LWI(i, c) (((((c)) & (WCOLS - 1)) << 5) + ((i) - (c)))
    const int r1 = r0 + B2;
    int ix, ixc[4], ib[4], id[4], it[4];
    if (FAST) {
        const int UB = ((c0 & (WCOLS - 1)) << 5) + (r0 - c0), UD = (r0 & (WCOLS - 1)) << 5;
        ix = UB + r;
        for (int j = 0; j < 4; ++j) {
            ixc[j] = UB + 4 * g + j;
            ib[j] = UB + cA + 31 * j;
            id[j] = UD + offD[j];
            it[j] = UD + cT + j;
        }
    } else {
        ix = LWI(r0 + r, c0);
        for (int j = 0; j < 4; ++j) {
            const int cc = 4 * g + j;
            ixc[j] = LWI(r0 + cc, c0);
            ib[j] = LWI(r0 + r, c0 + cc);
            id[j] = r >= cc ? LWI(r0 + r, r0 + cc) : LWI(r0 + cc, r0 + r);
            it[j] = LWI(r1 + cc, r0 + r);
        }
    }
#undef LWI
    const double x = Lw[ix];
    double xc[4], b[4], dv[4], bt[4];
    for (int j = 0; j < 4; ++j) {
        xc[j] = Lw[ixc[j]];
        b[j] = k > 0 ? Lw[ib[j]] : 0.0;
        dv[j] = Lw[id[j]];
        bt[j] = Lw[it[j]];
    }
    const double nrm2 = rsum16(r > 0 ? x * x : 0.0);
    const double alpha = read_lane(x, 0);
    double tq = 0.0, scale = 0.0, beta = alpha;
    if (nrm2 != 0.0) house_params(alpha, nrm2, beta, tq, scale);
    const double v = r == 0 ? 1.0 : x * scale;
    double vc[4];
    for (int j = 0; j < 4; ++j) vc[j] = (4 * g + j) == 0 ? 1.0 : xc[j] * scale;
    if (g == 0) Lw[ix] = r == 0 ? beta : 0.0;
    if (k > 0) {
        double d4[4];
        for (int j = 0; j < 4; ++j) d4[j] = v * b[j];
        rsum16x4(d4);
        for (int j = 0; j < 4; ++j)
            if (4 * g + j > 0) Lw[ib[j]] = b[j] - tq * d4[j] * v;
    }
    {
        double q4[4];
        for (int j = 0; j < 4; ++j) q4[j] = bt[j] * v;
        rsum16x4(q4);
        for (int j = 0; j < 4; ++j) {
            const double q = tq * q4[j];
            Lw[it[j]] = bt[j] - q * v;
        }
    }
    double pc[4], part = 0.0;
    for (int j = 0; j < 4; ++j) pc[j] = v * dv[j];
    rsum16x4(pc);
    for (int j = 0; j < 4; ++j) {
        pc[j] = tq * pc[j];
        part += vc[j] * pc[j];
    }
    if (r < 4) pS[4 * g + r] = r == 0 ? pc[0] : (r == 1 ? pc[1] : (r == 2 ? pc[2] : pc[3]));
    const double vtp = (read_lane(part, 0) + read_lane(part, 16)) + (read_lane(part, 32) + read_lane(part, 48));
    const double kk = 0.5 * tq * vtp;
    const double w = pS[r] - kk * v;
    for (int j = 0; j < 4; ++j) {
        const double wc = pc[j] - kk * vc[j];
        if (r >= 4 * g + j) Lw[id[j]] = dv[j] - v * wc - w * vc[j];
    }
}

struct Sb16Ctl {
    unsigned long long hs;
    int err, pad;
    unsigned long long prog[8];
};
constexpr unsigned long long S16_COMMIT = 1ull << 62, S16_ABORT = 1ull << 63;

__device__ __forceinline__ void s16_wait(const unsigned long long *pollp, unsigned long long want, Sb16Ctl *C, int *status)
{
    int spin = 0;
    const int bound = __hip_atomic_load(&C->err, __ATOMIC_RELAXED, __HIP_MEMORY_SCOPE_AGENT) ? 2000 : 20000000;
    while (__hip_atomic_load(pollp, __ATOMIC_RELAXED, __HIP_MEMORY_SCOPE_AGENT) < want) {
        if (++spin > bound) {
            atomicExch(&C->err, 1);
            if (status) atomicExch(status, BSP_ERR_HIP);
            break;
        }
        if ((spin & 1023) == 0 && __hip_atomic_load(&C->err, __ATOMIC_RELAXED, __HIP_MEMORY_SCOPE_AGENT)) break;
        __builtin_amdgcn_s_sleep(2);
    }
    asm volatile("buffer_inv sc1" ::: "memory");
}

__global__ __launch_bounds__(576) void sb16st_kernel(int n, int npad, int batch, double *__restrict__ ABall,
                                                     double *__restrict__ dall, double *__restrict__ eall, long long *diag,
                                                     Sb16Ctl *ctl, int P, int *status, int force_abort)
{
    extern __shared__ double lds[];
    double *Lw = lds;
    long long dacc[5] = {0, 0, 0, 0, 0}, dt0 = 0;
    const int tid = threadIdx.x, lane = tid & 63, wv = __builtin_amdgcn_readfirstlane(tid >> 6);
    const int r = lane & 15, g = lane >> 4;
    double *pS = lds + WCOLS * WROWS + (wv & 7) * 16;
    const int cA = 124 * g + r, cT = 31 * r + 4 * g + 16;
    int offD[4];
    for (int j = 0; j < 4; ++j) offD[j] = r >= 4 * g + j ? cA + 31 * j : 31 * r + 4 * g + j;
    int chn = blockIdx.x, w = 0, stride = 1;
    const unsigned long long *pollp = nullptr;
    unsigned long long *pubp = nullptr;
    Sb16Ctl *C = nullptr;
    if (ctl) {
        const int blk = blockIdx.x, grp = blk / (8 * P), rr = blk % (8 * P);
        chn = grp * 8 + (rr & 7); w = rr >> 3;
        if (chn >= batch) return;
        C = ctl + chn;
        int *modep = reinterpret_cast<int *>(lds + WCOLS * WROWS + NW2 * 16);
        if (tid == 0) {
            const unsigned long long xcc = (unsigned long long)(__builtin_amdgcn_s_getreg((31 << 11) | 20) & 0xfu);
            const unsigned long long mine = (0x10ull | xcc) << (8 * w);
            unsigned long long full = 0;
            for (int q = 0; q < P; ++q) full |= 0x10ull << (8 * q);
            unsigned long long v = atomicOr(&C->hs, mine) | mine;
            for (int spin = 0; !(v & (S16_COMMIT | S16_ABORT)); ++spin) {
                if (force_abort == 1) atomicCAS(&C->hs, v, v | S16_ABORT);
                else if ((v & full) == full) atomicCAS(&C->hs, v, v | S16_COMMIT);
                else if (spin > 400000) atomicCAS(&C->hs, v, v | S16_ABORT);
                else __builtin_amdgcn_s_sleep(4);
                v = __hip_atomic_load(&C->hs, __ATOMIC_RELAXED, __HIP_MEMORY_SCOPE_AGENT);
            }
            int mode;
            if (v & S16_ABORT) mode = (w == 0) ? 2 : 0;
            else {
                bool same = true;
                for (int q = 1; q < P; ++q) same = same && (((v >> (8 * q)) & 0xfu) == (v & 0xfu));
                if (force_abort == 2) same = false;
                mode = same ? 1 : ((w == 0) ? 2 : 0);
            }
            *modep = mode;
        }
        __syncthreads();
        const int mode = __builtin_amdgcn_readfirstlane(*modep);
        __syncthreads();
        if (mode == 0) return;
        if (mode == 1 && P > 1) { stride = P; pollp = &C->prog[(w + P - 1) % P]; pubp = &C->prog[w]; }
        else w = 0;
    }
    double *AB = ABall + (size_t)chn * ab_stride(npad);
#define LW(i, c) Lw[((((c)) & (WCOLS - 1)) << 5) + ((i) - (c))]

    double *dump = AB + (size_t)npad * LD + 64;
    const int npass = (n - 2 + NW2 - 1) / NW2;
    for (int ps = w; ps < npass; ps += stride) {
        const int s0 = ps * NW2;
        int RP = s0, LP = s0 + 64;
        if (pollp && ps > 0) {
            if (tid == 0) {
                const int need = s0 + 128 < n ? s0 + 128 : n;
                s16_wait(pollp, ((unsigned long long)(ps - 1) << 32) + (unsigned)need, C, status);
            }
            __syncthreads();
            asm volatile("buffer_inv sc1" ::: "memory");
        }
        for (int idx = tid; idx < 64 * WROWS; idx += 576) {
            const int c = s0 + (idx >> 5), d = idx & 31;
            Lw[((c & (WCOLS - 1)) << 5) + d] = c + d < n ? AB[(size_t)c * LD + d] : 0.0;
        }
        const int md = lane & 31, mh = lane >> 5;
        double qb[32];
        unsigned long long pw = 0;
        if (wv == NW2) {
            const unsigned o0 = (unsigned)(LP + mh) * LD + md, omax = (unsigned)(n - 1) * LD;
            for (int i = 0; i < 32; ++i) {
                unsigned o = o0 + 2 * LD * i;
                o = o < omax ? o : omax;
                qb[i] = AB[o];
            }
        }
        __syncthreads();
        const int s = s0 + wv;
        const int nsteps = (n - s0 - 1 + B2 - 1) / B2 + LAG * (NW2 - 1);
        for (int t = 0; t < nsteps; ++t) {
            int RPn = s0 + NW2 + B2 * (t - LAG * (NW2 - 1) - 1);
            if (RPn > n) RPn = n;
            if (RPn < RP) RPn = RP;
            if (wv == NW2) {
                if (diag) dt0 = (long long)__builtin_amdgcn_s_memtime();
                if ((t & 3) == 0) {
                    if (pollp && ps > 0 && LP + 64 < n) {
                        const int need = LP + 128 < n ? LP + 128 : n;
                        const unsigned long long want = ((unsigned long long)(ps - 1) << 32) + (unsigned)need;
                        if (pw < want) s16_wait(pollp, want, C, status);
                        else asm volatile("buffer_inv sc1" ::: "memory");
                    }
                    {
                        const unsigned s0_ = (unsigned)(LP + mh), lim = (unsigned)(n - md);
                        for (int i = 0; i < 32; ++i) {
                            const unsigned c = s0_ + 2 * i;
                            Lw[(((c & (WCOLS - 1)) << 5) + md)] = c < lim ? qb[i] : 0.0;
                        }
                        const unsigned o0 = (unsigned)(LP + 64 + mh) * LD + md, omax = (unsigned)(n - 1) * LD;
                        for (int i = 0; i < 32; ++i) {
                            unsigned o = o0 + 2 * LD * i;
                            o = o < omax ? o : omax;
                            qb[i] = AB[o];
                        }
                    }
                }
                if ((t & 3) == 3 && pubp) {
                    asm volatile("s_waitcnt vmcnt(0)" ::: "memory");
                    if (lane == 0)
                        __hip_atomic_store(pubp, ((unsigned long long)ps << 32) + (unsigned)RP, __ATOMIC_RELAXED,
                                           __HIP_MEMORY_SCOPE_AGENT);
                }
                if ((t & 3) == 2 && pollp) pw = __hip_atomic_load(pollp, __ATOMIC_RELAXED, __HIP_MEMORY_SCOPE_AGENT);
                if (diag) { const long long t_ = (long long)__builtin_amdgcn_s_memtime(); dacc[1] += t_ - dt0; dt0 = t_; }
                {
                    const unsigned c0_ = (unsigned)(RP + mh), dumpo = (unsigned)npad * LD + 64 + lane;
                    for (int i = 0; i < 8; ++i) {
                        const unsigned c = c0_ + 2 * i;
                        const unsigned o = c < (unsigned)RPn ? c * LD + md : dumpo;
                        AB[o] = Lw[((c & (WCOLS - 1)) << 5) + md];
                    }
                }
                if (diag) { const long long t_ = (long long)__builtin_amdgcn_s_memtime(); dacc[0] += t_ - dt0; }
            }
            if ((t & 3) == 0) LP += 64;
            RP = RPn;
            const int k = t - LAG * wv;
            const int r0 = s + 1 + B2 * k;
            if (diag) dt0 = (long long)__builtin_amdgcn_s_memtime();
            if (wv < NW2 && k >= 0 && s < n - 2 && r0 < n) {
                const int c0 = k == 0 ? s : r0 - B2;
                const bool fast = (c0 & (WCOLS - 1)) <= WCOLS - 16 && (r0 & (WCOLS - 1)) <= WCOLS - 16;
                if (fast) chase_item<true>(Lw, pS, r0, c0, k, r, g, cA, cT, offD);
                else chase_item<false>(Lw, pS, r0, c0, k, r, g, cA, cT, offD);
                if (diag) { asm volatile("s_waitcnt lgkmcnt(0)" ::: "memory"); const long long t_ = (long long)__builtin_amdgcn_s_memtime(); dacc[2] += t_ - dt0; dt0 = t_; }
            }
            lds_barrier();
            if (diag) { const long long t_ = (long long)__builtin_amdgcn_s_memtime(); dacc[3] += t_ - dt0; dacc[4] += 1; }
        }
        __syncthreads();
        int hi = LP < n ? LP : n;
        for (int idx = tid; idx < (hi - RP) * WROWS; idx += 576) {
            const int c = RP + (idx >> 5), d = idx & 31;
            AB[(size_t)c * LD + d] = Lw[((c & (WCOLS - 1)) << 5) + d];
        }
        __syncthreads();
        if (pubp && tid == 0)
            __hip_atomic_store(pubp, ((unsigned long long)ps << 32) + (unsigned)n, __ATOMIC_RELAXED, __HIP_MEMORY_SCOPE_AGENT);
    }
#undef LW
    if (diag && blockIdx.x == 0 && lane == 0)
        for (int q = 0; q < 5; ++q) diag[wv * 5 + q] = dacc[q];
    if (stride > 1 && (npass - 1) % stride != w && npass > 0) return;
    __syncthreads();
    asm volatile("buffer_inv sc1" ::: "memory");
    double *dd = dall + (size_t)chn * npad, *ee = eall + (size_t)chn * npad;
    for (int j = tid; j < n; j += 576) {
        dd[j] = AB[(size_t)j * LD];
        ee[j] = j < n - 1 ? AB[(size_t)j * LD + 1] : 0.0;
    }
}

constexpr int NCW4 = 6, SB16R_THREADS = (NCW4 + 1) * 64;
constexpr int SBR_MLAG_SHORT = 2;
__device__ __forceinline__ double &ldsb(double *Lw, int off) { return *reinterpret_cast<double *>(reinterpret_cast<char *>(Lw) + off); }

template <int B>
struct Rw {
    static constexpr int WR = 2 * B;
    static constexpr int WSH = B == 16 ? 5 : 4;
    static constexpr int RPW = 64 / B;
    static constexpr int NSW = 2 * RPW;
    static constexpr int MLAG = B == 16 ? 4 : 8;
    static constexpr int LP0 = B * (MLAG + 3);
    static constexpr int MLAGS = B == 16 ? MLAG : SBR_MLAG_SHORT;
    static constexpr int STAGGER = LAG * NSW + 2 * MLAG + 5;
    static constexpr int Z = WCOLS * WR;
    static constexpr int DUMP = Z + 128;
    static constexpr int XS = DUMP + 384;
    static constexpr int XPAR = NSW * 2 * B;
    static constexpr int MODE = XS + 2 * XPAR;
    static constexpr int LDS = (MODE + 2) * 8;
    static_assert(B == 16 || B == 8, "tile sizes of the rows kernel");
    static_assert((1 << WSH) == WR && XPAR == 256 && LP0 + B <= 128, "window layout");
};

template <int B>
__device__ __forceinline__ double rsumB(double x)
{
    x += dpp_mov<0xB1>(x);
    x += dpp_mov<0x4E>(x);
    x += dpp_mov<0x141>(x);
    if (B == 16) x += dpp_mov<0x140>(x);
    return x;
}
template <int B>
__device__ __forceinline__ void rsumBx2(double &a, double &b)
{
    a += dpp_mov<0xB1>(a); b += dpp_mov<0xB1>(b);
    a += dpp_mov<0x4E>(a); b += dpp_mov<0x4E>(b);
    a += dpp_mov<0x141>(a); b += dpp_mov<0x141>(b);
    if (B == 16) { a += dpp_mov<0x140>(a); b += dpp_mov<0x140>(b); }
}

template <int B>
__device__ __forceinline__ void next_reflector(double *Lw, const double x0, const int j, const int xw, const int hx)
{
    double nrm2 = j > 0 ? x0 * x0 : 0.0, alpha = j == 0 ? x0 : 0.0;
    rsumBx2<B>(nrm2, alpha);
    const bool nz = nrm2 != 0.0;
    const double beta0 = -copysign(sqrt(fma(alpha, alpha, nz ? nrm2 : 1.0)), alpha);
    const double tq0 = (beta0 - alpha) / beta0, scale0 = 1.0 / (alpha - beta0);
    const double beta = nz ? beta0 : alpha, tq = nz ? tq0 : 0.0, scale = nz ? scale0 : 0.0;
    Lw[xw + j] = j == 0 ? 1.0 : x0 * scale;
    if (j == 0) Lw[xw + B] = tq;
    ldsb(Lw, hx) = j == 0 ? beta : 0.0;
}

template <int B, bool FAST>
__device__ __forceinline__ void next_tile_addr(const int r0, const int j, int (&at)[B])
{
    const int cb = r0 & (WCOLS - 1), a0 = ((cb << Rw<B>::WSH) + B + j) * 8, iw = WCOLS - cb;
#pragma unroll
    for (int i = 0; i < B; ++i) at[i] = (FAST || i < iw) ? a0 : a0 - WCOLS * Rw<B>::WR * 8;
}
template <int B, bool FAST>
__device__ __forceinline__ void diag_tile_addr(const int r0, const int j, const int (&offD)[B], int (&ad)[B])
{
    const int cb = r0 & (WCOLS - 1), ud = (cb << Rw<B>::WSH) * 8, iw = WCOLS - cb, udq = j >= iw ? ud - WCOLS * Rw<B>::WR * 8 : ud;
#pragma unroll
    for (int i = 0; i < B; ++i) ad[i] = ((!FAST && i >= iw) ? udq : ud) + offD[i];
}

template <int B>
__device__ __forceinline__ void chase4_next(double *Lw, double (&bt)[B], const double (&v)[B], const double tq, const int (&at)[B],
                                            const int j, const int xw)
{
    double y0 = bt[0], y1 = v[1] * bt[1], y2 = v[2] * bt[2], y3 = v[3] * bt[3];
#pragma unroll
    for (int i = 4; i < B; i += 4) {
        y0 = fma(v[i], bt[i], y0); y1 = fma(v[i + 1], bt[i + 1], y1);
        y2 = fma(v[i + 2], bt[i + 2], y2); y3 = fma(v[i + 3], bt[i + 3], y3);
    }
    const double ct = tq * ((y0 + y1) + (y2 + y3));
    next_reflector<B>(Lw, bt[0] - ct, j, xw, at[0]);
#pragma unroll
    for (int i = 1; i < B; ++i) ldsb(Lw, at[i] + (Rw<B>::WR - 1) * 8 * i) = fma(-ct, v[i], bt[i]);
}

template <int B>
__device__ __forceinline__ void chase4_diag(double *Lw, const double (&d)[B], const int (&ad)[B], const int j, const int xr,
                                            const int zi, const int dumpi)
{
    double v[B];
#pragma unroll
    for (int i = 0; i < B; ++i) v[i] = Lw[xr + i];
    const double tq = Lw[xr + B], vl = Lw[xr + j];
    double y0 = d[0], y1 = v[1] * d[1], y2 = v[2] * d[2], y3 = v[3] * d[3];
#pragma unroll
    for (int i = 4; i < B; i += 4) {
        y0 = fma(v[i], d[i], y0); y1 = fma(v[i + 1], d[i + 1], y1);
        y2 = fma(v[i + 2], d[i + 2], y2); y3 = fma(v[i + 3], d[i + 3], y3);
    }
    const double p = tq * ((y0 + y1) + (y2 + y3));
    const double vtp = rsumB<B>(vl * p);
    const double z = fma(-(0.5 * tq * vtp), vl, p);
    Lw[zi + j] = z;
    double zz[B];
#pragma unroll
    for (int i = 0; i < B; ++i) zz[i] = Lw[zi + i];
#pragma unroll
    for (int i = 0; i < B; ++i) ldsb(Lw, i >= j ? ad[i] : (dumpi + i) * 8) = fma(-zz[i], vl, fma(-v[i], z, d[i]));
}

template <int B>
__device__ __forceinline__ void chase4_bulge(double *Lw, const int r0, const int c0, const int j, const int xr, const int dumpi)
{
    double v[B], b[B];
#pragma unroll
    for (int i = 0; i < B; ++i) v[i] = Lw[xr + i];
    const double tq = Lw[xr + B];
    int ab = (((c0 + j) & (WCOLS - 1)) << Rw<B>::WSH) + (r0 - c0 - j);
    if (j == 0) ab = dumpi;
#pragma unroll
    for (int i = 0; i < B; ++i) b[i] = Lw[ab + i];
    double w0 = b[0], w1 = v[1] * b[1], w2 = v[2] * b[2], w3 = v[3] * b[3];
#pragma unroll
    for (int i = 4; i < B; i += 4) {
        w0 = fma(v[i], b[i], w0); w1 = fma(v[i + 1], b[i + 1], w1);
        w2 = fma(v[i + 2], b[i + 2], w2); w3 = fma(v[i + 3], b[i + 3], w3);
    }
    const double cb = tq * ((w0 + w1) + (w2 + w3));
#pragma unroll
    for (int i = 0; i < B; ++i) Lw[ab + i] = fma(-cb, v[i], b[i]);
}

__global__ void band_tail_zero_kernel(int n, int npad, int wr, double *__restrict__ ABall)
{
    double *AB = ABall + (size_t)blockIdx.x * ab_stride(npad);
    const int c_lo = n - (wr - 1) > 0 ? n - (wr - 1) : 0;
    for (int idx = threadIdx.x; idx < (npad + 1 - c_lo) * wr; idx += blockDim.x) {
        const int c = c_lo + idx / wr, d = idx % wr;
        if (c + d >= n) AB[(size_t)c * LD + d] = 0.0;
    }
}

template <int B, int PH, int MLAG>
__device__ __forceinline__ void mover_step(double *Lw, double *__restrict__ AB, const int n, const int npad, const int LP,
                                           const int RP, const int RPn, const int RPold, const int ps, const int lane,
                                           const unsigned long long *pollp, unsigned long long *pubp, unsigned long long &pw,
                                           unsigned long long &ptmp, Sb16Ctl *C, int *status, const bool diag, long long (&dacc)[5])
{
    constexpr int WSH = Rw<B>::WSH;
    long long ts = diag ? (long long)__builtin_amdgcn_s_memtime() : 0;
#define MV_STAMP(q) if (diag) { const long long t_ = (long long)__builtin_amdgcn_s_memtime(); dacc[q] += t_ - ts; ts = t_; }
    if (PH == 0 && pollp && ps > 0 && LP < n) {
        const int need = LP + 4 * B < n ? LP + 4 * B : n;
        const unsigned long long want = ((unsigned long long)(ps - 1) << 32) + (unsigned)need;
        if (pw < want) s16_wait(pollp, want, C, status);
        else asm volatile("buffer_inv sc1" ::: "memory");
    }
    if (B == 16) {
#pragma unroll
        for (int q = 0; q < 4; ++q) {
            const int c = LP + 4 * q, cl = c + (lane >> 4);
            const double *src = AB + (size_t)(cl < npad ? cl : npad) * LD + 2 * (lane & 15);
            double *dst = Lw + ((c & (WCOLS - 1)) << WSH);
            __builtin_amdgcn_global_load_lds((const __attribute__((address_space(1))) void *)src,
                                             (__attribute__((address_space(3))) void *)dst, 16, 0, 0);
        }
    } else {
        const int cl = LP + (lane >> 3);
        const double *src = AB + (size_t)(cl < npad ? cl : npad) * LD + 2 * (lane & 7);
        double *dst = Lw + ((LP & (WCOLS - 1)) << WSH);
        __builtin_amdgcn_global_load_lds((const __attribute__((address_space(1))) void *)src,
                                         (__attribute__((address_space(3))) void *)dst, 16, 0, 0);
    }
    if (PH == 1 && pollp) asm volatile("global_load_dwordx2 %0, %1, off sc1" : "+v"(ptmp) : "v"(pollp) : "memory");
    MV_STAMP(1)
    {
        const int md = lane & (Rw<B>::WR - 1), mh = lane >> WSH;
        const unsigned c0_ = (unsigned)(RP + mh), dumpo = (unsigned)npad * LD + 64 + lane;
#pragma unroll
        for (int i = 0; i < B * Rw<B>::WR / 64; ++i) {
            const unsigned c = c0_ + (64 / Rw<B>::WR) * i;
            const unsigned o = c < (unsigned)RPn ? c * LD + md : dumpo;
            AB[o] = Lw[((c & (WCOLS - 1)) << WSH) + md];
        }
    }
    MV_STAMP(0)
    constexpr int OPS = (B == 16 ? 12 : 3) * MLAG;
    constexpr bool SHORT = MLAG < Rw<B>::MLAG;
    constexpr int NPOLL = !SHORT ? 0 : (MLAG >= 4 ? MLAG / 4 : (((PH + 3) & 3) < MLAG ? 1 : 0));
    if (SHORT && NPOLL && pollp) asm volatile("s_waitcnt vmcnt(%0)" ::"n"(OPS + NPOLL) : "memory");
    else asm volatile("s_waitcnt vmcnt(%0)" ::"n"(OPS) : "memory");
    MV_STAMP(2)
#undef MV_STAMP
    if ((PH == 3 || (SHORT && PH == 1)) && pubp && lane == 0)
        __hip_atomic_store(pubp, ((unsigned long long)ps << 32) + (unsigned)RPold, __ATOMIC_RELAXED, __HIP_MEMORY_SCOPE_AGENT);
    if (PH == 3 && pollp) {
        const unsigned lo = __builtin_amdgcn_readfirstlane((unsigned)ptmp), hi = __builtin_amdgcn_readfirstlane((unsigned)(ptmp >> 32));
        pw = ((unsigned long long)hi << 32) | lo;
    }
}

template <int B>
__device__ __forceinline__ void stores_done_barrier()
{
    if (B == 16) asm volatile("s_waitcnt lgkmcnt(15)\n\ts_barrier" ::: "memory");
    else asm volatile("s_waitcnt lgkmcnt(7)\n\ts_barrier" ::: "memory");
}

template <int B, bool DIAG, int MLAG>
__device__ __forceinline__ void mover_pass(double *Lw, double *__restrict__ AB, const int n, const int npad, const int s0,
                                           const int nsteps, const int ps, const int lane, const unsigned long long *pollp,
                                           unsigned long long *pubp, Sb16Ctl *C, int *status, long long (&dacc)[5], long long *pd)
{
    constexpr int NSW = Rw<B>::NSW;
    unsigned long long pw = 0, ptmp = 0;
    int RP = s0, LP = s0 + B * (MLAG + 3), RPold = s0;
    long long dt0 = 0;
    const long long tp0 = DIAG ? (long long)__builtin_amdgcn_s_memtime() : 0, w0 = dacc[1];
#define SB16R_MSTEP(PH) \
    if (t + PH < nsteps) { \
        int RPn = s0 + NSW + B * ((t + PH) - LAG * (NSW - 1) - 1);    \
        if (RPn > n) RPn = n; \
        if (RPn < RP) RPn = RP; \
        { int r4 = s0 + NSW + B * ((t + PH - MLAG) - LAG * (NSW - 1) - 1);       \
          RPold = r4 > n ? n : (r4 < s0 ? s0 : r4); } \
        mover_step<B, PH, MLAG>(Lw, AB, n, npad, LP + B * PH, RP, RPn, RPold, ps, lane, pollp, pubp, pw, ptmp, C, status, DIAG, dacc); \
        if (DIAG) dt0 = (long long)__builtin_amdgcn_s_memtime(); \
        RP = RPn; \
        lds_barrier(); \
        if (DIAG) { const long long t_ = (long long)__builtin_amdgcn_s_memtime(); dacc[3] += t_ - dt0; dacc[4] += 1; } \
    }
    for (int t = 0; t < nsteps; t += 4) {
        SB16R_MSTEP(0) SB16R_MSTEP(1) SB16R_MSTEP(2) SB16R_MSTEP(3)
        LP += 4 * B;
    }
#undef SB16R_MSTEP
    asm volatile("s_waitcnt vmcnt(0)" ::: "memory");
    if (DIAG && pd && lane == 0) {
        pd[0] = nsteps; pd[1] = (long long)__builtin_amdgcn_s_memtime() - tp0; pd[2] = dacc[1] - w0;
    }
}

constexpr int SBR_PASSDIAG = 256;
template <int B, bool DIAG, bool PHASED>
__device__ __forceinline__ void sbr_rows_body(int n, int npad, int batch, double *__restrict__ ABall, double *__restrict__ dall,
                                              double *__restrict__ eall, long long *diag, Sb16Ctl *ctl, int P, int *status,
                                              int force_abort, int lagmode)
{
    using W = Rw<B>;
    constexpr int WSH = W::WSH, WR = W::WR, RPW = W::RPW, NSW = W::NSW, MLAG = W::MLAG, LP0 = W::LP0;
    constexpr int RINGB = WCOLS * WR * 8, STEPB = B * WR * 8;
    static_assert(!PHASED || B == 8, "the phased step loop is built for tiles of 8");
    extern __shared__ double lds[];
    double *Lw = lds;
    __builtin_amdgcn_s_setprio(3);
    long long dacc[5] = {0, 0, 0, 0, 0}, dt0 = 0;
    const int tid = threadIdx.x, lane = tid & 63, wv = __builtin_amdgcn_readfirstlane(tid >> 6);
    const int j = lane & (B - 1), g = lane / B;
    const int grp = wv < 4 ? (wv >> 1) & 1 : wv & 1, role = wv < 4 ? wv & 1 : 2, sw = RPW * grp + g;
    const int zi = W::Z + 64 * grp + B * g, dumpi = W::DUMP + 64 * (wv % NCW4) + B * g;
    int chn = blockIdx.x, w = 0, stride = 1;
    const unsigned long long *pollp = nullptr;
    unsigned long long *pubp = nullptr;
    Sb16Ctl *C = nullptr;
    if (ctl) {
        const int blk = blockIdx.x, grp = blk / (8 * P), rr = blk % (8 * P);
        chn = grp * 8 + (rr & 7); w = rr >> 3;
        if (chn >= batch) return;
        C = ctl + chn;
        int *modep = reinterpret_cast<int *>(lds + W::MODE);
        if (tid == 0) {
            const unsigned long long xcc = (unsigned long long)(__builtin_amdgcn_s_getreg((31 << 11) | 20) & 0xfu);
            const unsigned long long mine = (0x10ull | xcc) << (8 * w);
            unsigned long long full = 0;
            for (int q = 0; q < P; ++q) full |= 0x10ull << (8 * q);
            unsigned long long v = atomicOr(&C->hs, mine) | mine;
            for (int spin = 0; !(v & (S16_COMMIT | S16_ABORT)); ++spin) {
                if (force_abort == 1) atomicCAS(&C->hs, v, v | S16_ABORT);
                else if ((v & full) == full) atomicCAS(&C->hs, v, v | S16_COMMIT);
                else if (spin > 400000) atomicCAS(&C->hs, v, v | S16_ABORT);
                else __builtin_amdgcn_s_sleep(4);
                v = __hip_atomic_load(&C->hs, __ATOMIC_RELAXED, __HIP_MEMORY_SCOPE_AGENT);
            }
            int mode;
            if (v & S16_ABORT) mode = (w == 0) ? 2 : 0;
            else {
                bool same = true;
                for (int q = 1; q < P; ++q) same = same && (((v >> (8 * q)) & 0xfu) == (v & 0xfu));
                if (force_abort == 2) same = false;
                mode = same ? 1 : ((w == 0) ? 2 : 0);
            }
            *modep = mode;
        }
        __syncthreads();
        const int mode = __builtin_amdgcn_readfirstlane(*modep);
        __syncthreads();
        if (mode == 0) return;
        if (mode == 1 && P > 1) { stride = P; pollp = &C->prog[(w + P - 1) % P]; pubp = &C->prog[w]; }
        else w = 0;
    }
    double *AB = ABall + (size_t)chn * ab_stride(npad);
    const int npass = (n - 2 + NSW - 1) / NSW;
    for (int ps = w; ps < npass; ps += stride) {
        const int s0 = ps * NSW;
        const int nsteps = (n - s0 - 1 + B - 1) / B + LAG * (NSW - 1);
        const bool shortp = W::MLAGS < MLAG && (lagmode == 2 || (lagmode == 0 && stride > 1 && nsteps < stride * W::STAGGER));
        const int lp0 = shortp ? B * (W::MLAGS + 3) : LP0;
        int RP = s0, LP = s0 + lp0;
        const long long tw0 = DIAG ? (long long)__builtin_amdgcn_s_memtime() : 0;
        if (pollp && ps > 0) {
            if (tid == 0) {
                const int need = s0 + lp0 + B < n ? s0 + lp0 + B : n;
                s16_wait(pollp, ((unsigned long long)(ps - 1) << 32) + (unsigned)need, C, status);
            }
            __syncthreads();
            asm volatile("buffer_inv sc1" ::: "memory");
        }
        long long *pd = nullptr;
        if (DIAG && blockIdx.x == 0 && (ps - w) / stride < SBR_PASSDIAG) {
            pd = diag + 45 + 4 * ((ps - w) / stride);
            if (wv == NCW4 && lane == 0) pd[3] = (long long)__builtin_amdgcn_s_memtime() - tw0;
        }
        for (int idx = tid; idx < lp0 * WR; idx += SB16R_THREADS) {
            const int c = s0 + (idx >> WSH), d = idx & (WR - 1);
            Lw[((c & (WCOLS - 1)) << WSH) + d] = c + d < n ? AB[(size_t)c * LD + d] : 0.0;
        }
        __syncthreads();
        if (wv == 0 && g == 0) {
            const int hx = ((s0 & (WCOLS - 1)) << WSH) + 1 + j;
            next_reflector<B>(Lw, Lw[hx], j, W::XS, hx * 8);
        }
        if (wv == NCW4) {
            __syncthreads();
            if (shortp) mover_pass<B, DIAG, W::MLAGS>(Lw, AB, n, npad, s0, nsteps, ps, lane, pollp, pubp, C, status, dacc, pd);
            else mover_pass<B, DIAG, MLAG>(Lw, AB, n, npad, s0, nsteps, ps, lane, pollp, pubp, C, status, dacc, pd);
        } else {
            const int s4 = s0 + sw;
            const bool live = s4 < n - 2;
            const int xs0 = W::XS + sw * 2 * B;
            const int r04b = s4 + 1 - B * LAG * sw;
            int tA = nsteps, tB = nsteps;
            unsigned long long wmask = 0;
            if (PHASED) {
                const int sw0 = RPW * grp, x = n - s0 - 1 - B - sw0 + B * LAG * sw0;
                tA = LAG * (sw0 + RPW - 1);
                tB = s0 + sw0 + RPW - 1 < n - 2 && x > 0 ? (x - 1) / B + 1 : 0;
                if (tB > nsteps) tB = nsteps;
                if (tA > nsteps) tA = nsteps;
                if (tB < tA) tB = tA;
                const int basep = r04b + B + WCOLS;
                const int tw = (63 - (basep >> 3)) & 63, wr = (basep & 7) != 0;
#pragma unroll
                for (int q = 0; q < RPW; ++q) {
                    const int twq = __builtin_amdgcn_readlane(tw, B * q), wrq = __builtin_amdgcn_readlane(wr, B * q);
                    wmask |= (unsigned long long)wrq << twq;
                }
            }
            if (role == 0) {
                double bt[B], v[B], tq = 0.0;
                int at[B];
                for (int i = 0; i < B; ++i) { bt[i] = 0.0; v[i] = 0.0; at[i] = 0; }
                if (sw == 0 && live && s4 + 1 < n) {
                    next_tile_addr<B, false>(s4 + 1, j, at);
#pragma unroll
                    for (int i = 0; i < B; ++i) { bt[i] = ldsb(Lw, at[i] + (WR - 1) * 8 * i); v[i] = Lw[xs0 + i]; }
                    tq = Lw[xs0 + B];
                }
                __syncthreads();
                auto general_step = [&](const int t) {
                    if (DIAG) dt0 = (long long)__builtin_amdgcn_s_memtime();
                    const int k4 = t - LAG * sw, r04 = r04b + B * t;
                    const bool act = k4 >= 0 && live && r04 < n, actN = k4 >= -1 && live && r04 + B < n;
                    const int xw = xs0 + (((t + 1) & 1) << 8);
                    if (act) {
                        chase4_next<B>(Lw, bt, v, tq, at, j, xw);
                    } else if (k4 == -1 && live) {
                        const int hx = ((s4 & (WCOLS - 1)) << WSH) + 1 + j;
                        next_reflector<B>(Lw, Lw[hx], j, xw, hx * 8);
                    }
                    const bool wrapN = __builtin_amdgcn_ballot_w64(actN && ((r04 + B) & (WCOLS - 1)) > WCOLS - B) != 0;
                    if (actN) {
                        if (wrapN) next_tile_addr<B, false>(r04 + B, j, at);
                        else next_tile_addr<B, true>(r04 + B, j, at);
#pragma unroll
                        for (int i = 0; i < B; ++i) v[i] = Lw[xw + i];
                        tq = Lw[xw + B];
#pragma unroll
                        for (int i = 0; i < B; ++i) bt[i] = ldsb(Lw, at[i] + (WR - 1) * 8 * i);
                    }
                    if (DIAG) { const long long t_ = (long long)__builtin_amdgcn_s_memtime(); dacc[2] += t_ - dt0; dt0 = t_; }
                    if (__builtin_amdgcn_ballot_w64(actN) != 0) stores_done_barrier<B>();
                    else lds_barrier();
                    if (DIAG) { const long long t_ = (long long)__builtin_amdgcn_s_memtime(); dacc[3] += t_ - dt0; dacc[4] += 1; }
                };
                for (int t = 0; t < tA; ++t) general_step(t);
                if (PHASED && tB > tA) {
                    const unsigned long long wm2 = wmask | (wmask << 1) | (wmask >> 63);
                    int a0 = ((((r04b + B * tA) & (WCOLS - 1)) << WSH) + B + j) * 8;
                    int xw = xs0 + (((tA + 1) & 1) << 8);
                    for (int t = tA; t < tB; ++t) {
                        if (DIAG) dt0 = (long long)__builtin_amdgcn_s_memtime();
                        if (!((wm2 >> (t & 63)) & 1)) {
                            int af[B];
#pragma unroll
                            for (int i = 0; i < B; ++i) af[i] = a0;
                            chase4_next<B>(Lw, bt, v, tq, af, j, xw);
                            a0 = (a0 + STEPB) & (RINGB - 1);
#pragma unroll
                            for (int i = 0; i < B; ++i) v[i] = Lw[xw + i];
                            tq = Lw[xw + B];
#pragma unroll
                            for (int i = 0; i < B; ++i) bt[i] = ldsb(Lw, a0 + (WR - 1) * 8 * i);
                            asm volatile("; plain step" ::: "memory");
                        } else {
                            int ag[B];
                            const int r04 = r04b + B * t;
                            next_tile_addr<B, false>(r04, j, ag);
                            chase4_next<B>(Lw, bt, v, tq, ag, j, xw);
                            next_tile_addr<B, false>(r04 + B, j, ag);
                            a0 = (a0 + STEPB) & (RINGB - 1);
#pragma unroll
                            for (int i = 0; i < B; ++i) v[i] = Lw[xw + i];
                            tq = Lw[xw + B];
#pragma unroll
                            for (int i = 0; i < B; ++i) bt[i] = ldsb(Lw, ag[i] + (WR - 1) * 8 * i);
                            asm volatile("; wrapping step" ::: "memory");
                        }
                        xw ^= 256;
                        if (DIAG) { const long long t_ = (long long)__builtin_amdgcn_s_memtime(); dacc[2] += t_ - dt0; dt0 = t_; }
                        stores_done_barrier<B>();
                        if (DIAG) { const long long t_ = (long long)__builtin_amdgcn_s_memtime(); dacc[3] += t_ - dt0; dacc[4] += 1; }
                    }
                    next_tile_addr<B, false>(r04b + B * tB, j, at);
                }
                for (int t = tB; t < nsteps; ++t) general_step(t);
            } else if (role == 1) {
                double d[B];
                int ad[B], offD[B];
                int jo = j;
                if (PHASED) asm volatile("" : "+v"(jo));
                for (int i = 0; i < B; ++i) { d[i] = 0.0; ad[i] = 0; offD[i] = (i >= jo ? (WR - 1) * jo + i : (WR - 1) * i + jo) * 8; }
                if (sw == 0 && live && s4 + 1 < n) {
                    diag_tile_addr<B, false>(s4 + 1, j, offD, ad);
#pragma unroll
                    for (int i = 0; i < B; ++i) d[i] = ldsb(Lw, ad[i]);
                }
                __syncthreads();
                auto general_step = [&](const int t) {
                    if (DIAG) dt0 = (long long)__builtin_amdgcn_s_memtime();
                    const int k4 = t - LAG * sw, r04 = r04b + B * t;
                    const bool act = k4 >= 0 && live && r04 < n, actN = k4 >= -1 && live && r04 + B < n;
                    if (act) chase4_diag<B>(Lw, d, ad, j, xs0 + ((t & 1) << 8), zi, dumpi);
                    const bool wrapN = __builtin_amdgcn_ballot_w64(actN && ((r04 + B) & (WCOLS - 1)) > WCOLS - B) != 0;
                    if (actN) {
                        if (wrapN) diag_tile_addr<B, false>(r04 + B, j, offD, ad);
                        else diag_tile_addr<B, true>(r04 + B, j, offD, ad);
#pragma unroll
                        for (int i = 0; i < B; ++i) d[i] = ldsb(Lw, ad[i]);
                    }
                    if (DIAG) { const long long t_ = (long long)__builtin_amdgcn_s_memtime(); dacc[2] += t_ - dt0; dt0 = t_; }
                    if (__builtin_amdgcn_ballot_w64(actN) != 0) stores_done_barrier<B>();
                    else lds_barrier();
                    if (DIAG) { const long long t_ = (long long)__builtin_amdgcn_s_memtime(); dacc[3] += t_ - dt0; dacc[4] += 1; }
                };
                for (int t = 0; t < tA; ++t) general_step(t);
                if (PHASED && tB > tA) {
                    int ud = (((r04b + B * tA) & (WCOLS - 1)) << WSH) * 8;
                    int xr = xs0 + ((tA & 1) << 8);
                    for (int t = tA; t < tB; ++t) {
                        if (DIAG) dt0 = (long long)__builtin_amdgcn_s_memtime();
                        chase4_diag<B>(Lw, d, ad, j, xr, zi, dumpi);
                        ud = (ud + STEPB) & (RINGB - 1);
                        if ((wmask >> (t & 63)) & 1) {
                            diag_tile_addr<B, false>(r04b + B * (t + 1), j, offD, ad);
                        } else {
#pragma unroll
                            for (int i = 0; i < B; ++i) ad[i] = ud + offD[i];
                            asm volatile("; plain step" : "+v"(ad[0]), "+v"(ad[1]), "+v"(ad[2]), "+v"(ad[3]), "+v"(ad[4]), "+v"(ad[5]), "+v"(ad[6]), "+v"(ad[7]));
                        }
#pragma unroll
                        for (int i = 0; i < B; ++i) d[i] = ldsb(Lw, ad[i]);
                        xr ^= 256;
                        if (DIAG) { const long long t_ = (long long)__builtin_amdgcn_s_memtime(); dacc[2] += t_ - dt0; dt0 = t_; }
                        stores_done_barrier<B>();
                        if (DIAG) { const long long t_ = (long long)__builtin_amdgcn_s_memtime(); dacc[3] += t_ - dt0; dacc[4] += 1; }
                    }
                }
                for (int t = tB; t < nsteps; ++t) general_step(t);
            } else {
                __syncthreads();
                auto general_step = [&](const int t) {
                    if (DIAG) dt0 = (long long)__builtin_amdgcn_s_memtime();
                    const int k4 = t - LAG * sw, r04 = r04b + B * t;
                    if (k4 > 0 && live && r04 < n) chase4_bulge<B>(Lw, r04, r04 - B, j, xs0 + ((t & 1) << 8), dumpi);
                    if (DIAG) { asm volatile("s_waitcnt lgkmcnt(0)" ::: "memory"); const long long t_ = (long long)__builtin_amdgcn_s_memtime(); dacc[2] += t_ - dt0; dt0 = t_; }
                    lds_barrier();
                    if (DIAG) { const long long t_ = (long long)__builtin_amdgcn_s_memtime(); dacc[3] += t_ - dt0; dacc[4] += 1; }
                };
                const int tA2 = tA + 1 < tB ? tA + 1 : tB;
                for (int t = 0; t < tA2; ++t) general_step(t);
                if (PHASED && tB > tA2) {
                    int r04 = r04b + B * tA2, xr = xs0 + ((tA2 & 1) << 8);
                    for (int t = tA2; t < tB; ++t) {
                        if (DIAG) dt0 = (long long)__builtin_amdgcn_s_memtime();
                        chase4_bulge<B>(Lw, r04, r04 - B, j, xr, dumpi);
                        r04 += B; xr ^= 256;
                        if (DIAG) { asm volatile("s_waitcnt lgkmcnt(0)" ::: "memory"); const long long t_ = (long long)__builtin_amdgcn_s_memtime(); dacc[2] += t_ - dt0; dt0 = t_; }
                        lds_barrier();
                        if (DIAG) { const long long t_ = (long long)__builtin_amdgcn_s_memtime(); dacc[3] += t_ - dt0; dacc[4] += 1; }
                    }
                }
                for (int t = tB; t < nsteps; ++t) general_step(t);
            }
        }
        if (nsteps > 0) {
            int RPn = s0 + NSW + B * ((nsteps - 1) - LAG * (NSW - 1) - 1);
            if (RPn > n) RPn = n;
            if (RPn < RP) RPn = RP;
            RP = RPn;
        }
        LP += 4 * B * ((nsteps + 3) / 4);
        __syncthreads();
        int hi = LP < n ? LP : n;
        for (int idx = tid; idx < (hi - RP) * WR; idx += SB16R_THREADS) {
            const int c = RP + (idx >> WSH), d = idx & (WR - 1);
            AB[(size_t)c * LD + d] = Lw[((c & (WCOLS - 1)) << WSH) + d];
        }
        __syncthreads();
        if (pubp && tid == 0)
            __hip_atomic_store(pubp, ((unsigned long long)ps << 32) + (unsigned)n, __ATOMIC_RELAXED, __HIP_MEMORY_SCOPE_AGENT);
    }
    if (DIAG && blockIdx.x == 0 && lane == 0)
        for (int q = 0; q < 5; ++q) diag[wv * 5 + q] = dacc[q];
    if (stride > 1 && (npass - 1) % stride != w && npass > 0) return;
    __syncthreads();
    asm volatile("buffer_inv sc1" ::: "memory");
    double *dd = dall + (size_t)chn * npad, *ee = eall + (size_t)chn * npad;
    for (int jj = tid; jj < n; jj += SB16R_THREADS) {
        dd[jj] = AB[(size_t)jj * LD];
        ee[jj] = jj < n - 1 ? AB[(size_t)jj * LD + 1] : 0.0;
    }
}

#define SBR_ROWS_ARGS int n, int npad, int batch, double *__restrict__ ABall, double *__restrict__ dall, double *__restrict__ eall, \
                      long long *diag, Sb16Ctl *ctl, int P, int *status, int force_abort, int lagmode
template <int B, bool DIAG = false>
__global__ __launch_bounds__(SB16R_THREADS) __attribute__((amdgpu_waves_per_eu(B == 8 ? 4 : 2))) void sbr_rows_kernel(SBR_ROWS_ARGS)
{
    sbr_rows_body<B, DIAG, B == 8>(n, npad, batch, ABall, dall, eall, diag, ctl, P, status, force_abort, lagmode);
}
template <int B, bool DIAG = false>
__global__ __launch_bounds__(SB16R_THREADS) __attribute__((amdgpu_waves_per_eu(B == 8 ? 4 : 2))) void sbr_rows_general_kernel(SBR_ROWS_ARGS)
{
    sbr_rows_body<B, DIAG, false>(n, npad, batch, ABall, dall, eall, diag, ctl, P, status, force_abort, lagmode);
}
#undef SBR_ROWS_ARGS

}

int launch_sb2sb(int n, int npad, int batch, double *d_AB, hipStream_t st)
{
    static bool attr = false;
    if (!attr) {
        BSP_HIP(allow_lds(sb2sb_kernel, SB2SB_LDS));
        BSP_HIP(allow_lds(sb2sb_mfma_kernel, SB2SB2_LDS));
        attr = true;
    }
    const int mf = opts().sb2sb_mfma;
    if (opts().sb2st_diag) {
        int nb1 = 0, nb2 = 0;
        hipOccupancyMaxActiveBlocksPerMultiprocessor(&nb1, reinterpret_cast<const void *>(sb2sb_mfma_kernel), 256, SB2SB2_LDS);
        hipOccupancyMaxActiveBlocksPerMultiprocessor(&nb2, reinterpret_cast<const void *>(sb2sb_kernel), 256, SB2SB_LDS);
        fprintf(stderr, "sb2sb: workgroups per CU by the occupancy query: mfma kernel %d (LDS %d B), first kernel %d (LDS %d B)\n", nb1,
                SB2SB2_LDS, nb2, SB2SB_LDS);
    }
    const int S = (n - NB1 + NB1 - 1) / NB1;
    auto K = [n](int s) { const int m = n - (NB1 * s + NB1); return m > 0 ? (m + B1 - 1) / B1 : 0; };
    int tmax = -1;
    for (int s = 0; s < S; ++s)
        if (K(s) > 0 && K(s) - 1 + LAG * s > tmax) tmax = K(s) - 1 + LAG * s;
    for (int t = 0; t <= tmax; ++t) {
        int s_hi = t / LAG;
        if (s_hi > S - 1) s_hi = S - 1;
        if (t - LAG * s_hi >= K(s_hi)) continue;
        int s_lo = s_hi;
        while (s_lo > 0 && t - LAG * (s_lo - 1) < K(s_lo - 1)) --s_lo;
        KScope kt(KS_SB2SB, st);
        if (mf) hipLaunchKernelGGL(sb2sb_mfma_kernel, dim3(s_hi - s_lo + 1, batch), dim3(256), SB2SB2_LDS, st, n, npad, d_AB, t, s_lo);
        else hipLaunchKernelGGL(sb2sb_kernel, dim3(s_hi - s_lo + 1, batch), dim3(256), SB2SB_LDS, st, n, npad, d_AB, t, s_lo);
    }
    BSP_HIP(hipGetLastError());
    return BSP_OK;
}

int launch_sb16st(int n, int npad, int batch, double *d_AB, double *d_d, double *d_e, hipStream_t st, int *d_status, void *ctl, int hb)
{
    static bool attr = false;
    static int wg8 = 1;
    if (!attr) {
        BSP_HIP(allow_lds(sb16st_kernel, SB16_LDS));
        BSP_HIP(allow_lds(sbr_rows_kernel<16, false>, Rw<16>::LDS));
        BSP_HIP(allow_lds(sbr_rows_kernel<16, true>, Rw<16>::LDS));
        BSP_HIP(allow_lds(sbr_rows_kernel<8, false>, Rw<8>::LDS));
        BSP_HIP(allow_lds(sbr_rows_kernel<8, true>, Rw<8>::LDS));
        BSP_HIP(allow_lds(sbr_rows_general_kernel<8, false>, Rw<8>::LDS));
        BSP_HIP(allow_lds(sbr_rows_general_kernel<8, true>, Rw<8>::LDS));
        int nb = 0;
        if (hipOccupancyMaxActiveBlocksPerMultiprocessor(&nb, reinterpret_cast<const void *>(sbr_rows_kernel<8, false>), SB16R_THREADS,
                                                         Rw<8>::LDS) == hipSuccess && nb >= 1) wg8 = nb > 2 ? 2 : nb;
        attr = true;
    }
    if (hb != 16 && hb != 8) return BSP_ERR_ARG;
    const bool rows = hb == 8 || opts().sb16_rows != 0;
    const int nsw = hb == 8 ? Rw<8>::NSW : NW2;
    int P;
    if (opts().sb2st_ring > 0) P = opts().sb2st_ring;
    else if (hb == 16) P = batch > 128 ? 1 : (batch > 64 ? 2 : (batch > 32 ? 4 : 8));
    else {
        const int cus = device_cus();
        const int wgs = opts().sb8_wgs > 0 && opts().sb8_wgs < wg8 ? opts().sb8_wgs : wg8;
        for (P = 8; P > 1 && ((batch + 7) / 8) * 8 * P > cus; P /= 2) {}
        if (P < 4 && opts().sb8_wgs == 0)
            for (P = 4; P > 1 && ((batch + 7) / 8) * 8 * P > cus * wgs; P /= 2) {}
        else if (opts().sb8_wgs > 0)
            for (P = 8; P > 1 && ((batch + 7) / 8) * 8 * P > cus * wgs; P /= 2) {}
    }
    if (P > 8) P = 8;
    while (P > 1 && (n - 2) / nsw < 2 * P) P /= 2;
    Sb16Ctl *d_ctl = nullptr;
    static_assert(sizeof(Sb16Ctl) <= 112, "the caller's per-problem control block is sized for sb2st.hip's Sb8Ctl (112 bytes per channel)");
    if (P > 1) {
        if (!ctl) return BSP_ERR_ARG;
        d_ctl = static_cast<Sb16Ctl *>(ctl);
        BSP_HIP(hipMemsetAsync(d_ctl, 0, (size_t)batch * sizeof(Sb16Ctl), st));
    }
    const int nblk = P > 1 ? ((batch + 7) / 8) * 8 * P : batch;
    const int fab = opts().sb2st_force_abort;
    const bool phased = opts().sbr_phased != 0;
    const int lagmode = opts().sbr_lag;
    auto launch = [&](long long *dbuf) {
        if (rows) hipLaunchKernelGGL(band_tail_zero_kernel, dim3(batch), dim3(256), 0, st, n, npad, 2 * hb, d_AB);
#define SBR_LAUNCH(K, ...) hipLaunchKernelGGL((K<__VA_ARGS__>), dim3(nblk), dim3(SB16R_THREADS), Rw<8>::LDS, st, n, npad, batch, d_AB, d_d, d_e, dbuf, \
                                              d_ctl, P, d_status, fab, lagmode)
        if (hb == 8 && dbuf && phased) SBR_LAUNCH(sbr_rows_kernel, 8, true);
        else if (hb == 8 && dbuf) SBR_LAUNCH(sbr_rows_general_kernel, 8, true);
        else if (hb == 8 && phased) SBR_LAUNCH(sbr_rows_kernel, 8, false);
        else if (hb == 8) SBR_LAUNCH(sbr_rows_general_kernel, 8, false);
#undef SBR_LAUNCH
        else if (rows && dbuf)
            hipLaunchKernelGGL((sbr_rows_kernel<16, true>), dim3(nblk), dim3(SB16R_THREADS), Rw<16>::LDS, st, n, npad, batch, d_AB, d_d, d_e, dbuf,
                               d_ctl, P, d_status, fab, 1);
        else if (rows)
            hipLaunchKernelGGL((sbr_rows_kernel<16, false>), dim3(nblk), dim3(SB16R_THREADS), Rw<16>::LDS, st, n, npad, batch, d_AB, d_d, d_e, dbuf,
                               d_ctl, P, d_status, fab, 1);
        else
            hipLaunchKernelGGL(sb16st_kernel, dim3(nblk), dim3(576), SB16_LDS, st, n, npad, batch, d_AB, d_d, d_e, dbuf, d_ctl, P,
                               d_status, fab);
    };
    if (opts().sb2st_diag) {
        static long long h[45 + 4 * SBR_PASSDIAG];
        long long *dbuf = nullptr;
        BSP_HIP(hipMalloc(reinterpret_cast<void **>(&dbuf), sizeof(h)));
        BSP_HIP(hipMemsetAsync(dbuf, 0, sizeof(h), st));
        launch(dbuf);
        const hipError_t le = hipGetLastError();
        if (le != hipSuccess) { hipFree(dbuf); BSP_HIP(le); }
        BSP_HIP(hipStreamSynchronize(st));
        BSP_HIP(hipMemcpy(h, dbuf, sizeof(h), hipMemcpyDeviceToHost));
        hipFree(dbuf);
        fprintf(stderr, "band chase, tiles of %d: %d workgroup(s) per channel, %d per CU\n", hb, P, hb == 8 ? wg8 : 1);
        for (int w = 0; w < 9; ++w) {
            const double steps = h[w * 5 + 4] > 0 ? (double)h[w * 5 + 4] : 1.0;
            fprintf(stderr, "sb16st wave %d: %lld steps; s_memtime ticks per step: chase item %.0f, rest + barrier %.0f (mover wave: columns out %.0f, block in %.0f)\n",
                    w, h[w * 5 + 4], (double)h[w * 5 + 2] / steps, (double)h[w * 5 + 3] / steps, (double)h[w * 5] / steps,
                    (double)h[w * 5 + 1] / steps);
        }
        for (int q = 0; q < SBR_PASSDIAG && h[45 + 4 * q] > 0; ++q) {
            const long long *pq = h + 45 + 4 * q;
            const double tick = (double)pq[1] / (double)pq[0];
            fprintf(stderr, "sb16st pass %d of workgroup 0: %lld steps, %.0f ticks per step; waited %.1f steps for its start, %.1f steps in poll check + requests\n",
                    q, pq[0], tick, (double)pq[3] / tick, (double)pq[2] / tick);
        }
        return BSP_OK;
    }
    KScope kt(KS_SB16ST, st);
    launch(nullptr);
    BSP_HIP(hipGetLastError());
    return BSP_OK;
}

}
```

Measured before the change: 2112 eigensolves/s.

## Use DPP row-broadcast FMAs for bulge-chasing reflector updates in band reduction

Adds inline-assembly DPP forms (v_fmac_f64_dpp with row_newbcast) that apply the 8-wide Householder dot and axpy/rank-2 updates in the band-to-tridiagonal chase, broadcasting the reflector lane instead of reloading the full reflector vector from LDS. It also switches the phased kernel to absolute LDS addressing. A new option selects levels 0-3, defaulting to 2, which changes the diagonal-tile update to a fused rank-2 DPP update and avoids the z round-trip through LDS. This is meant to cut LDS traffic and latency on the serial chase path, at the cost of hand-written ISA, added nop padding and a changed summation order.

```diff
diff --git a/bspatom_amd/csrc/capi.hip b/bspatom_amd/csrc/capi.hip
--- a/bspatom_amd/csrc/capi.hip
+++ b/bspatom_amd/csrc/capi.hip
@@ -103,6 +103,7 @@
     {"sb8_wgs", "BSP_SB8_WGS", &Options::sb8_wgs},
     {"sbr_phased", "BSP_SBR_PHASED", &Options::sbr_phased},
     {"sbr_lag", "BSP_SBR_LAG", &Options::sbr_lag},
+    {"sbr_xdpp", "BSP_SBR_XDPP", &Options::sbr_xdpp},
     {"fused_probe", "BSP_FUSED_PROBE", &Options::fused_probe},
     {"dipole_stage_mb", "BSP_DIPOLE_STAGE_MB", &Options::dipole_stage_mb},
     {"resolvent_stage_mb", "BSP_RESOLVENT_STAGE_MB", &Options::resolvent_stage_mb},
diff --git a/bspatom_amd/csrc/common.h b/bspatom_amd/csrc/common.h
--- a/bspatom_amd/csrc/common.h
+++ b/bspatom_amd/csrc/common.h
@@ -26,6 +26,8 @@
 __host__ __device__ inline size_t ab_stride(int npad) { return (size_t)npad * 128 + 1088; }
 
 namespace bsp {
+
+constexpr int SBR_XDPP_DEFAULT = 2;
 
 struct Options {
     int sb2st_version = 0;
@@ -66,6 +68,7 @@
     int sb8_wgs = 0;
     int sbr_phased = 1;
     int sbr_lag = 0;
+    int sbr_xdpp = SBR_XDPP_DEFAULT;
     int cw_ipw = 0;
     int cw_ldspad = 0;
     int cw_onediv = 0;
diff --git a/bspatom_amd/csrc/sbr2.hip b/bspatom_amd/csrc/sbr2.hip
--- a/bspatom_amd/csrc/sbr2.hip
+++ b/bspatom_amd/csrc/sbr2.hip
@@ -706,6 +706,11 @@
 constexpr int NCW4 = 6, SB16R_THREADS = (NCW4 + 1) * 64;
 constexpr int SBR_MLAG_SHORT = 2;
 __device__ __forceinline__ double &ldsb(double *Lw, int off) { return *reinterpret_cast<double *>(reinterpret_cast<char *>(Lw) + off); }
+typedef __attribute__((address_space(3))) double lds_f64;
+__device__ __forceinline__ int lds_addr(double *Lw) { return (int)(size_t)(__attribute__((address_space(3))) double *)Lw; }
+__device__ __forceinline__ double &ldsa(int addr) { return *(double *)(lds_f64 *)(size_t)(unsigned)addr; }
+template <bool ABS>
+__device__ __forceinline__ double &ldsx(double *Lw, int off) { return ABS ? ldsa(off) : ldsb(Lw, off); }
 
 template <int B>
 struct Rw {
@@ -746,17 +751,69 @@
 }
 
 template <int B>
-__device__ __forceinline__ void next_reflector(double *Lw, const double x0, const int j, const int xw, const int hx)
+__device__ __forceinline__ void next_reflector(double *Lw, const double x0, const int j, const int xw, const int hx, double &vlo, double &tqo)
 {
     double nrm2 = j > 0 ? x0 * x0 : 0.0, alpha = j == 0 ? x0 : 0.0;
     rsumBx2<B>(nrm2, alpha);
     const bool nz = nrm2 != 0.0;
     const double beta0 = -copysign(sqrt(fma(alpha, alpha, nz ? nrm2 : 1.0)), alpha);
     const double tq0 = (beta0 - alpha) / beta0, scale0 = 1.0 / (alpha - beta0);
-    const double beta = nz ? beta0 : alpha, tq = nz ? tq0 : 0.0, scale = nz ? scale0 : 0.0;
-    Lw[xw + j] = j == 0 ? 1.0 : x0 * scale;
+    const double beta = nz ? beta0 : alpha, scale = nz ? scale0 : 0.0;
+    double tq = nz ? tq0 : 0.0;
+    asm volatile("" : "+v"(tq));
+    const double vl = j == 0 ? 1.0 : x0 * scale;
+    Lw[xw + j] = vl;
     if (j == 0) Lw[xw + B] = tq;
     ldsb(Lw, hx) = j == 0 ? beta : 0.0;
+    vlo = vl; tqo = tq;
+}
+template <int B>
+__device__ __forceinline__ void next_reflector(double *Lw, const double x0, const int j, const int xw, const int hx)
+{
+    double vl, tq;
+    next_reflector<B>(Lw, x0, j, xw, hx, vl, tq);
+}
+
+#define XD_PAD "s_nop 1\n\t"
+#define XD_LO " row_mask:0xf bank_mask:0x3\n\t"
+#define XD_HI " row_mask:0xf bank_mask:0xc\n\t"
+#define XD_FL(k, s, m) "v_fmac_f64_dpp %[a" #k "], %[" #s "], " m " row_newbcast:" #k XD_LO
+#define XD_FH(k, s, m) "v_fmac_f64_dpp %[a" #k "], %[" #s "], " m " row_newbcast:%[u" #k "]" XD_HI
+#define XD_DL(y, k) "v_fmac_f64_dpp %[y" #y "], %[vl], %[x" #k "] row_newbcast:" #k XD_LO
+#define XD_DH(y, k) "v_fmac_f64_dpp %[y" #y "], %[vl], %[x" #k "] row_newbcast:%[u" #k "]" XD_HI
+#define XD_U [u0] "i"(8), [u1] "i"(9), [u2] "i"(10), [u3] "i"(11), [u4] "i"(12), [u5] "i"(13), [u6] "i"(14), [u7] "i"(15)
+#define XD_A(k) [a##k] "+v"(a[k])
+#define XD_F7(s, m) XD_FL(1, s, m) XD_FL(2, s, m) XD_FL(3, s, m) XD_FL(4, s, m) XD_FL(5, s, m) XD_FL(6, s, m) XD_FL(7, s, m) \
+                    XD_FH(1, s, m) XD_FH(2, s, m) XD_FH(3, s, m) XD_FH(4, s, m) XD_FH(5, s, m) XD_FH(6, s, m) XD_FH(7, s, m)
+#define XD_F8(s, m) XD_FL(0, s, m) XD_FL(1, s, m) XD_FL(2, s, m) XD_FL(3, s, m) XD_FL(4, s, m) XD_FL(5, s, m) XD_FL(6, s, m) XD_FL(7, s, m) \
+                    XD_FH(0, s, m) XD_FH(1, s, m) XD_FH(2, s, m) XD_FH(3, s, m) XD_FH(4, s, m) XD_FH(5, s, m) XD_FH(6, s, m) XD_FH(7, s, m)
+
+__device__ __forceinline__ double xd_dot(const double vl, const double (&x)[8])
+{
+    double y0 = x[0], y1 = -0.0, y2 = -0.0, y3 = -0.0;
+    asm(XD_PAD XD_DL(1, 1) XD_DL(2, 2) XD_DL(3, 3) XD_DL(0, 4) XD_DL(1, 5) XD_DL(2, 6) XD_DL(3, 7)
+        XD_DH(1, 1) XD_DH(2, 2) XD_DH(3, 3) XD_DH(0, 4) XD_DH(1, 5) XD_DH(2, 6) XD_DH(3, 7)
+        : [y0] "+v"(y0), [y1] "+v"(y1), [y2] "+v"(y2), [y3] "+v"(y3)
+        : [vl] "v"(vl), [x1] "v"(x[1]), [x2] "v"(x[2]), [x3] "v"(x[3]), [x4] "v"(x[4]), [x5] "v"(x[5]), [x6] "v"(x[6]), [x7] "v"(x[7]), XD_U);
+    return (y0 + y1) + (y2 + y3);
+}
+template <int FROM>
+__device__ __forceinline__ void xd_axpy(double (&a)[8], const double vl, const double c)
+{
+    static_assert(FROM == 0 || FROM == 1, "the whole tile, or all but its first element");
+    if constexpr (FROM == 0)
+        asm(XD_PAD XD_F8(s, "-%[c]") : XD_A(0), XD_A(1), XD_A(2), XD_A(3), XD_A(4), XD_A(5), XD_A(6), XD_A(7) : [s] "v"(vl), [c] "v"(c), XD_U);
+    else
+        asm(XD_PAD XD_F7(s, "-%[c]") : XD_A(1), XD_A(2), XD_A(3), XD_A(4), XD_A(5), XD_A(6), XD_A(7) : [s] "v"(vl), [c] "v"(c), XD_U);
+}
+template <bool INNER>
+__device__ __forceinline__ void xd_rank2(double (&a)[8], const double vl, const double z)
+{
+    if constexpr (INNER)
+        asm(XD_PAD XD_F8(vl, "-%[z]") XD_F8(z, "-%[vl]") : XD_A(0), XD_A(1), XD_A(2), XD_A(3), XD_A(4), XD_A(5), XD_A(6), XD_A(7)
+            : [vl] "v"(vl), [z] "v"(z), XD_U);
+    else
+        asm(XD_PAD XD_F8(z, "-%[vl]") : XD_A(0), XD_A(1), XD_A(2), XD_A(3), XD_A(4), XD_A(5), XD_A(6), XD_A(7) : [vl] "v"(vl), [z] "v"(z), XD_U);
 }
 
 template <int B, bool FAST>
@@ -774,67 +831,113 @@
     for (int i = 0; i < B; ++i) ad[i] = ((!FAST && i >= iw) ? udq : ud) + offD[i];
 }
 
-template <int B>
-__device__ __forceinline__ void chase4_next(double *Lw, double (&bt)[B], const double (&v)[B], const double tq, const int (&at)[B],
+template <int B, bool XD>
+__device__ __forceinline__ void chase4_next(double *Lw, double (&bt)[B], const double (&v)[B], double &vl, double &tq, const int (&at)[B],
                                             const int j, const int xw)
 {
-    double y0 = bt[0], y1 = v[1] * bt[1], y2 = v[2] * bt[2], y3 = v[3] * bt[3];
-#pragma unroll
-    for (int i = 4; i < B; i += 4) {
-        y0 = fma(v[i], bt[i], y0); y1 = fma(v[i + 1], bt[i + 1], y1);
-        y2 = fma(v[i + 2], bt[i + 2], y2); y3 = fma(v[i + 3], bt[i + 3], y3);
-    }
-    const double ct = tq * ((y0 + y1) + (y2 + y3));
-    next_reflector<B>(Lw, bt[0] - ct, j, xw, at[0]);
-#pragma unroll
-    for (int i = 1; i < B; ++i) ldsb(Lw, at[i] + (Rw<B>::WR - 1) * 8 * i) = fma(-ct, v[i], bt[i]);
-}
-
-template <int B>
+    if constexpr (XD) {
+        static_assert(B == 8, "the DPP forms are built for tiles of 8");
+        const double ct = tq * xd_dot(vl, bt);
+        const double x0 = bt[0] - ct;
+        xd_axpy<1>(bt, vl, ct);
+        next_reflector<B>(Lw, x0, j, xw, at[0], vl, tq);
+#pragma unroll
+        for (int i = 1; i < B; ++i) ldsb(Lw, at[i] + (Rw<B>::WR - 1) * 8 * i) = bt[i];
+    } else {
+        double y0 = bt[0], y1 = v[1] * bt[1], y2 = v[2] * bt[2], y3 = v[3] * bt[3];
+#pragma unroll
+        for (int i = 4; i < B; i += 4) {
+            y0 = fma(v[i], bt[i], y0); y1 = fma(v[i + 1], bt[i + 1], y1);
+            y2 = fma(v[i + 2], bt[i + 2], y2); y3 = fma(v[i + 3], bt[i + 3], y3);
+        }
+        const double ct = tq * ((y0 + y1) + (y2 + y3));
+        next_reflector<B>(Lw, bt[0] - ct, j, xw, at[0]);
+#pragma unroll
+        for (int i = 1; i < B; ++i) ldsb(Lw, at[i] + (Rw<B>::WR - 1) * 8 * i) = fma(-ct, v[i], bt[i]);
+    }
+}
+
+template <int B, int XD, bool ABS>
 __device__ __forceinline__ void chase4_diag(double *Lw, const double (&d)[B], const int (&ad)[B], const int j, const int xr,
-                                            const int zi, const int dumpi)
-{
-    double v[B];
-#pragma unroll
-    for (int i = 0; i < B; ++i) v[i] = Lw[xr + i];
-    const double tq = Lw[xr + B], vl = Lw[xr + j];
-    double y0 = d[0], y1 = v[1] * d[1], y2 = v[2] * d[2], y3 = v[3] * d[3];
-#pragma unroll
-    for (int i = 4; i < B; i += 4) {
-        y0 = fma(v[i], d[i], y0); y1 = fma(v[i + 1], d[i + 1], y1);
-        y2 = fma(v[i + 2], d[i + 2], y2); y3 = fma(v[i + 3], d[i + 3], y3);
-    }
-    const double p = tq * ((y0 + y1) + (y2 + y3));
-    const double vtp = rsumB<B>(vl * p);
-    const double z = fma(-(0.5 * tq * vtp), vl, p);
-    Lw[zi + j] = z;
-    double zz[B];
-#pragma unroll
-    for (int i = 0; i < B; ++i) zz[i] = Lw[zi + i];
-#pragma unroll
-    for (int i = 0; i < B; ++i) ldsb(Lw, i >= j ? ad[i] : (dumpi + i) * 8) = fma(-zz[i], vl, fma(-v[i], z, d[i]));
-}
-
-template <int B>
+                                            const int zi, const int dumpb)
+{
+    if constexpr (XD >= 2) {
+        static_assert(B == 8, "the DPP forms are built for tiles of 8");
+        const double tq = Lw[xr + B], vl = Lw[xr + j];
+        const double p = tq * xd_dot(vl, d);
+        const double vtp = rsumB<B>(vl * p);
+        const double z = fma(-(0.5 * tq * vtp), vl, p);
+        double a[B];
+#pragma unroll
+        for (int i = 0; i < B; ++i) a[i] = d[i];
+        xd_rank2<true>(a, vl, z);
+#pragma unroll
+        for (int i = 0; i < B; ++i) ldsx<ABS>(Lw, i >= j ? ad[i] : dumpb + 8 * i) = a[i];
+    } else {
+        double v[B];
+#pragma unroll
+        for (int i = 0; i < B; ++i) v[i] = Lw[xr + i];
+        const double tq = Lw[xr + B], vl = Lw[xr + j];
+        double y0 = d[0], y1 = v[1] * d[1], y2 = v[2] * d[2], y3 = v[3] * d[3];
+#pragma unroll
+        for (int i = 4; i < B; i += 4) {
+            y0 = fma(v[i], d[i], y0); y1 = fma(v[i + 1], d[i + 1], y1);
+            y2 = fma(v[i + 2], d[i + 2], y2); y3 = fma(v[i + 3], d[i + 3], y3);
+        }
+        const double p = tq * ((y0 + y1) + (y2 + y3));
+        const double vtp = rsumB<B>(vl * p);
+        const double z = fma(-(0.5 * tq * vtp), vl, p);
+        if constexpr (XD == 1) {
+            static_assert(B == 8, "the DPP forms are built for tiles of 8");
+            double a[B];
+#pragma unroll
+            for (int i = 0; i < B; ++i) a[i] = fma(-v[i], z, d[i]);
+            xd_rank2<false>(a, vl, z);
+#pragma unroll
+            for (int i = 0; i < B; ++i) ldsx<ABS>(Lw, i >= j ? ad[i] : dumpb + 8 * i) = a[i];
+        } else {
+            Lw[zi + j] = z;
+            double zz[B];
+#pragma unroll
+            for (int i = 0; i < B; ++i) zz[i] = Lw[zi + i];
+#pragma unroll
+            for (int i = 0; i < B; ++i) ldsx<ABS>(Lw, i >= j ? ad[i] : dumpb + 8 * i) = fma(-zz[i], vl, fma(-v[i], z, d[i]));
+        }
+    }
+}
+
+template <int B, bool XD>
 __device__ __forceinline__ void chase4_bulge(double *Lw, const int r0, const int c0, const int j, const int xr, const int dumpi)
 {
-    double v[B], b[B];
-#pragma unroll
-    for (int i = 0; i < B; ++i) v[i] = Lw[xr + i];
-    const double tq = Lw[xr + B];
+    double b[B];
     int ab = (((c0 + j) & (WCOLS - 1)) << Rw<B>::WSH) + (r0 - c0 - j);
     if (j == 0) ab = dumpi;
-#pragma unroll
-    for (int i = 0; i < B; ++i) b[i] = Lw[ab + i];
-    double w0 = b[0], w1 = v[1] * b[1], w2 = v[2] * b[2], w3 = v[3] * b[3];
-#pragma unroll
-    for (int i = 4; i < B; i += 4) {
-        w0 = fma(v[i], b[i], w0); w1 = fma(v[i + 1], b[i + 1], w1);
-        w2 = fma(v[i + 2], b[i + 2], w2); w3 = fma(v[i + 3], b[i + 3], w3);
-    }
-    const double cb = tq * ((w0 + w1) + (w2 + w3));
-#pragma unroll
-    for (int i = 0; i < B; ++i) Lw[ab + i] = fma(-cb, v[i], b[i]);
+    if constexpr (XD) {
+        static_assert(B == 8, "the DPP forms are built for tiles of 8");
+        const double tq = Lw[xr + B], vl = Lw[xr + j];
+#pragma unroll
+        for (int i = 0; i < B; ++i) b[i] = Lw[ab + i];
+        const double cb = tq * xd_dot(vl, b);
+        xd_axpy<0>(b, vl, cb);
+#pragma unroll
+        for (int i = 0; i < B; ++i) Lw[ab + i] = b[i];
+    } else {
+        double v[B];
+#pragma unroll
+        for (int i = 0; i < B; ++i) v[i] = Lw[xr + i];
+        const double tq = Lw[xr + B];
+#pragma unroll
+        for (int i = 0; i < B; ++i) b[i] = Lw[ab + i];
+        double w0 = b[0], w1 = v[1] * b[1], w2 = v[2] * b[2], w3 = v[3] * b[3];
+#pragma unroll
+        for (int i = 4; i < B; i += 4) {
+            w0 = fma(v[i], b[i], w0); w1 = fma(v[i + 1], b[i + 1], w1);
+            w2 = fma(v[i + 2], b[i + 2], w2); w3 = fma(v[i + 3], b[i + 3], w3);
+        }
+        const double cb = tq * ((w0 + w1) + (w2 + w3));
+#pragma unroll
+        for (int i = 0; i < B; ++i) Lw[ab + i] = fma(-cb, v[i], b[i]);
+    }
 }
 
 __global__ void band_tail_zero_kernel(int n, int npad, int wr, double *__restrict__ ABall)
@@ -906,10 +1009,12 @@
     }
 }
 
-template <int B>
+template <int B, int NLOADS = 0>
 __device__ __forceinline__ void stores_done_barrier()
 {
-    if (B == 16) asm volatile("s_waitcnt lgkmcnt(15)\n\ts_barrier" ::: "memory");
+    static_assert(NLOADS >= 0 && NLOADS <= 16, "lgkmcnt is a four-bit counter");
+    if (NLOADS > 0) asm volatile("s_waitcnt lgkmcnt(%0)\n\ts_barrier" ::"n"(NLOADS - 1) : "memory");
+    else if (B == 16) asm volatile("s_waitcnt lgkmcnt(15)\n\ts_barrier" ::: "memory");
     else asm volatile("s_waitcnt lgkmcnt(7)\n\ts_barrier" ::: "memory");
 }
 
@@ -948,7 +1053,7 @@
 }
 
 constexpr int SBR_PASSDIAG = 256;
-template <int B, bool DIAG, bool PHASED>
+template <int B, bool DIAG, bool PHASED, int XDPP>
 __device__ __forceinline__ void sbr_rows_body(int n, int npad, int batch, double *__restrict__ ABall, double *__restrict__ dall,
                                               double *__restrict__ eall, long long *diag, Sb16Ctl *ctl, int P, int *status,
                                               int force_abort, int lagmode)
@@ -957,8 +1062,12 @@
     constexpr int WSH = W::WSH, WR = W::WR, RPW = W::RPW, NSW = W::NSW, MLAG = W::MLAG, LP0 = W::LP0;
     constexpr int RINGB = WCOLS * WR * 8, STEPB = B * WR * 8;
     static_assert(!PHASED || B == 8, "the phased step loop is built for tiles of 8");
+    static_assert(XDPP >= 0 && XDPP <= 3 && (XDPP == 0 || B == 8), "the DPP forms are built for tiles of 8");
+    constexpr bool XD0 = XDPP >= 3;
+    constexpr bool ABS = PHASED;
     extern __shared__ double lds[];
     double *Lw = lds;
+    const int lb = ABS ? lds_addr(Lw) : 0;
     __builtin_amdgcn_s_setprio(3);
     long long dacc[5] = {0, 0, 0, 0, 0}, dt0 = 0;
     const int tid = threadIdx.x, lane = tid & 63, wv = __builtin_amdgcn_readfirstlane(tid >> 6);
@@ -1063,14 +1172,18 @@
                 }
             }
             if (role == 0) {
-                double bt[B], v[B], tq = 0.0;
+                double bt[B], v[B], tq = 0.0, vl = 0.0;
                 int at[B];
                 for (int i = 0; i < B; ++i) { bt[i] = 0.0; v[i] = 0.0; at[i] = 0; }
                 if (sw == 0 && live && s4 + 1 < n) {
                     next_tile_addr<B, false>(s4 + 1, j, at);
 #pragma unroll
-                    for (int i = 0; i < B; ++i) { bt[i] = ldsb(Lw, at[i] + (WR - 1) * 8 * i); v[i] = Lw[xs0 + i]; }
+                    for (int i = 0; i < B; ++i) {
+                        bt[i] = ldsb(Lw, at[i] + (WR - 1) * 8 * i);
+                        if (!XD0) v[i] = Lw[xs0 + i];
+                    }
                     tq = Lw[xs0 + B];
+                    if (XD0) vl = Lw[xs0 + j];
                 }
                 __syncthreads();
                 auto general_step = [&](const int t) {
@@ -1079,23 +1192,26 @@
                     const bool act = k4 >= 0 && live && r04 < n, actN = k4 >= -1 && live && r04 + B < n;
                     const int xw = xs0 + (((t + 1) & 1) << 8);
                     if (act) {
-                        chase4_next<B>(Lw, bt, v, tq, at, j, xw);
+                        chase4_next<B, XD0>(Lw, bt, v, vl, tq, at, j, xw);
                     } else if (k4 == -1 && live) {
                         const int hx = ((s4 & (WCOLS - 1)) << WSH) + 1 + j;
-                        next_reflector<B>(Lw, Lw[hx], j, xw, hx * 8);
+                        if (XD0) next_reflector<B>(Lw, Lw[hx], j, xw, hx * 8, vl, tq);
+                        else next_reflector<B>(Lw, Lw[hx], j, xw, hx * 8);
                     }
                     const bool wrapN = __builtin_amdgcn_ballot_w64(actN && ((r04 + B) & (WCOLS - 1)) > WCOLS - B) != 0;
                     if (actN) {
                         if (wrapN) next_tile_addr<B, false>(r04 + B, j, at);
                         else next_tile_addr<B, true>(r04 + B, j, at);
-#pragma unroll
-                        for (int i = 0; i < B; ++i) v[i] = Lw[xw + i];
-                        tq = Lw[xw + B];
+                        if (!XD0) {
+#pragma unroll
+                            for (int i = 0; i < B; ++i) v[i] = Lw[xw + i];
+                            tq = Lw[xw + B];
+                        }
 #pragma unroll
                         for (int i = 0; i < B; ++i) bt[i] = ldsb(Lw, at[i] + (WR - 1) * 8 * i);
                     }
                     if (DIAG) { const long long t_ = (long long)__builtin_amdgcn_s_memtime(); dacc[2] += t_ - dt0; dt0 = t_; }
-                    if (__builtin_amdgcn_ballot_w64(actN) != 0) stores_done_barrier<B>();
+                    if (__builtin_amdgcn_ballot_w64(actN) != 0) stores_done_barrier<B, XD0 ? 4 : 0>();
                     else lds_barrier();
                     if (DIAG) { const long long t_ = (long long)__builtin_amdgcn_s_memtime(); dacc[3] += t_ - dt0; dacc[4] += 1; }
                 };
@@ -1110,11 +1226,13 @@
                             int af[B];
 #pragma unroll
                             for (int i = 0; i < B; ++i) af[i] = a0;
-                            chase4_next<B>(Lw, bt, v, tq, af, j, xw);
+                            chase4_next<B, XD0>(Lw, bt, v, vl, tq, af, j, xw);
                             a0 = (a0 + STEPB) & (RINGB - 1);
-#pragma unroll
-                            for (int i = 0; i < B; ++i) v[i] = Lw[xw + i];
-                            tq = Lw[xw + B];
+                            if (!XD0) {
+#pragma unroll
+                                for (int i = 0; i < B; ++i) v[i] = Lw[xw + i];
+                                tq = Lw[xw + B];
+                            }
 #pragma unroll
                             for (int i = 0; i < B; ++i) bt[i] = ldsb(Lw, a0 + (WR - 1) * 8 * i);
                             asm volatile("; plain step" ::: "memory");
@@ -1122,19 +1240,21 @@
                             int ag[B];
                             const int r04 = r04b + B * t;
                             next_tile_addr<B, false>(r04, j, ag);
-                            chase4_next<B>(Lw, bt, v, tq, ag, j, xw);
+                            chase4_next<B, XD0>(Lw, bt, v, vl, tq, ag, j, xw);
                             next_tile_addr<B, false>(r04 + B, j, ag);
                             a0 = (a0 + STEPB) & (RINGB - 1);
-#pragma unroll
-                            for (int i = 0; i < B; ++i) v[i] = Lw[xw + i];
-                            tq = Lw[xw + B];
+                            if (!XD0) {
+#pragma unroll
+                                for (int i = 0; i < B; ++i) v[i] = Lw[xw + i];
+                                tq = Lw[xw + B];
+                            }
 #pragma unroll
                             for (int i = 0; i < B; ++i) bt[i] = ldsb(Lw, ag[i] + (WR - 1) * 8 * i);
                             asm volatile("; wrapping step" ::: "memory");
                         }
                         xw ^= 256;
                         if (DIAG) { const long long t_ = (long long)__builtin_amdgcn_s_memtime(); dacc[2] += t_ - dt0; dt0 = t_; }
-                        stores_done_barrier<B>();
+                        stores_done_barrier<B, XD0 ? 4 : 0>();
                         if (DIAG) { const long long t_ = (long long)__builtin_amdgcn_s_memtime(); dacc[3] += t_ - dt0; dacc[4] += 1; }
                     }
                     next_tile_addr<B, false>(r04b + B * tB, j, at);
@@ -1145,24 +1265,25 @@
                 int ad[B], offD[B];
                 int jo = j;
                 if (PHASED) asm volatile("" : "+v"(jo));
-                for (int i = 0; i < B; ++i) { d[i] = 0.0; ad[i] = 0; offD[i] = (i >= jo ? (WR - 1) * jo + i : (WR - 1) * i + jo) * 8; }
+                for (int i = 0; i < B; ++i) { d[i] = 0.0; ad[i] = 0; offD[i] = (i >= jo ? (WR - 1) * jo + i : (WR - 1) * i + jo) * 8 + lb; }
+                const int dumpb = dumpi * 8 + lb;
                 if (sw == 0 && live && s4 + 1 < n) {
                     diag_tile_addr<B, false>(s4 + 1, j, offD, ad);
 #pragma unroll
-                    for (int i = 0; i < B; ++i) d[i] = ldsb(Lw, ad[i]);
+                    for (int i = 0; i < B; ++i) d[i] = ldsx<ABS>(Lw, ad[i]);
                 }
                 __syncthreads();
                 auto general_step = [&](const int t) {
                     if (DIAG) dt0 = (long long)__builtin_amdgcn_s_memtime();
                     const int k4 = t - LAG * sw, r04 = r04b + B * t;
                     const bool act = k4 >= 0 && live && r04 < n, actN = k4 >= -1 && live && r04 + B < n;
-                    if (act) chase4_diag<B>(Lw, d, ad, j, xs0 + ((t & 1) << 8), zi, dumpi);
+                    if (act) chase4_diag<B, XDPP < 2 ? XDPP : 2, ABS>(Lw, d, ad, j, xs0 + ((t & 1) << 8), zi, dumpb);
                     const bool wrapN = __builtin_amdgcn_ballot_w64(actN && ((r04 + B) & (WCOLS - 1)) > WCOLS - B) != 0;
                     if (actN) {
                         if (wrapN) diag_tile_addr<B, false>(r04 + B, j, offD, ad);
                         else diag_tile_addr<B, true>(r04 + B, j, offD, ad);
 #pragma unroll
-                        for (int i = 0; i < B; ++i) d[i] = ldsb(Lw, ad[i]);
+                        for (int i = 0; i < B; ++i) d[i] = ldsx<ABS>(Lw, ad[i]);
                     }
                     if (DIAG) { const long long t_ = (long long)__builtin_amdgcn_s_memtime(); dacc[2] += t_ - dt0; dt0 = t_; }
                     if (__builtin_amdgcn_ballot_w64(actN) != 0) stores_done_barrier<B>();
@@ -1175,7 +1296,7 @@
                     int xr = xs0 + ((tA & 1) << 8);
                     for (int t = tA; t < tB; ++t) {
                         if (DIAG) dt0 = (long long)__builtin_amdgcn_s_memtime();
-                        chase4_diag<B>(Lw, d, ad, j, xr, zi, dumpi);
+                        chase4_diag<B, XDPP < 2 ? XDPP : 2, ABS>(Lw, d, ad, j, xr, zi, dumpb);
                         ud = (ud + STEPB) & (RINGB - 1);
                         if ((wmask >> (t & 63)) & 1) {
                             diag_tile_addr<B, false>(r04b + B * (t + 1), j, offD, ad);
@@ -1185,7 +1306,7 @@
                             asm volatile("; plain step" : "+v"(ad[0]), "+v"(ad[1]), "+v"(ad[2]), "+v"(ad[3]), "+v"(ad[4]), "+v"(ad[5]), "+v"(ad[6]), "+v"(ad[7]));
                         }
 #pragma unroll
-                        for (int i = 0; i < B; ++i) d[i] = ldsb(Lw, ad[i]);
+                        for (int i = 0; i < B; ++i) d[i] = ldsx<ABS>(Lw, ad[i]);
                         xr ^= 256;
                         if (DIAG) { const long long t_ = (long long)__builtin_amdgcn_s_memtime(); dacc[2] += t_ - dt0; dt0 = t_; }
                         stores_done_barrier<B>();
@@ -1198,7 +1319,7 @@
                 auto general_step = [&](const int t) {
                     if (DIAG) dt0 = (long long)__builtin_amdgcn_s_memtime();
                     const int k4 = t - LAG * sw, r04 = r04b + B * t;
-                    if (k4 > 0 && live && r04 < n) chase4_bulge<B>(Lw, r04, r04 - B, j, xs0 + ((t & 1) << 8), dumpi);
+                    if (k4 > 0 && live && r04 < n) chase4_bulge<B, XD0>(Lw, r04, r04 - B, j, xs0 + ((t & 1) << 8), dumpi);
                     if (DIAG) { asm volatile("s_waitcnt lgkmcnt(0)" ::: "memory"); const long long t_ = (long long)__builtin_amdgcn_s_memtime(); dacc[2] += t_ - dt0; dt0 = t_; }
                     lds_barrier();
                     if (DIAG) { const long long t_ = (long long)__builtin_amdgcn_s_memtime(); dacc[3] += t_ - dt0; dacc[4] += 1; }
@@ -1209,7 +1330,7 @@
                     int r04 = r04b + B * tA2, xr = xs0 + ((tA2 & 1) << 8);
                     for (int t = tA2; t < tB; ++t) {
                         if (DIAG) dt0 = (long long)__builtin_amdgcn_s_memtime();
-                        chase4_bulge<B>(Lw, r04, r04 - B, j, xr, dumpi);
+                        chase4_bulge<B, XD0>(Lw, r04, r04 - B, j, xr, dumpi);
                         r04 += B; xr ^= 256;
                         if (DIAG) { asm volatile("s_waitcnt lgkmcnt(0)" ::: "memory"); const long long t_ = (long long)__builtin_amdgcn_s_memtime(); dacc[2] += t_ - dt0; dt0 = t_; }
                         lds_barrier();
@@ -1253,12 +1374,23 @@
 template <int B, bool DIAG = false>
 __global__ __launch_bounds__(SB16R_THREADS) __attribute__((amdgpu_waves_per_eu(B == 8 ? 4 : 2))) void sbr_rows_kernel(SBR_ROWS_ARGS)
 {
-    sbr_rows_body<B, DIAG, B == 8>(n, npad, batch, ABall, dall, eall, diag, ctl, P, status, force_abort, lagmode);
+    sbr_rows_body<B, DIAG, B == 8, B == 8 ? SBR_XDPP_DEFAULT : 0>(n, npad, batch, ABall, dall, eall, diag, ctl, P, status, force_abort, lagmode);
+}
+template <bool DIAG, int XDPP>
+__global__ __launch_bounds__(SB16R_THREADS) __attribute__((amdgpu_waves_per_eu(4))) void sbr_rows_xdpp_kernel(SBR_ROWS_ARGS)
+{
+    sbr_rows_body<8, DIAG, true, XDPP>(n, npad, batch, ABall, dall, eall, diag, ctl, P, status, force_abort, lagmode);
 }
 template <int B, bool DIAG = false>
 __global__ __launch_bounds__(SB16R_THREADS) __attribute__((amdgpu_waves_per_eu(B == 8 ? 4 : 2))) void sbr_rows_general_kernel(SBR_ROWS_ARGS)
 {
-    sbr_rows_body<B, DIAG, false>(n, npad, batch, ABall, dall, eall, diag, ctl, P, status, force_abort, lagmode);
+    sbr_rows_body<B, DIAG, false, 0>(n, npad, batch, ABall, dall, eall, diag, ctl, P, status, force_abort, lagmode);
+}
+template <bool DIAG, int XDPP>
+auto sbr_rows8_kernel()
+{
+    if constexpr (XDPP == SBR_XDPP_DEFAULT) return &sbr_rows_kernel<8, DIAG>;
+    else return &sbr_rows_xdpp_kernel<DIAG, XDPP>;
 }
 #undef SBR_ROWS_ARGS
 
@@ -1307,8 +1439,14 @@
         BSP_HIP(allow_lds(sb16st_kernel, SB16_LDS));
         BSP_HIP(allow_lds(sbr_rows_kernel<16, false>, Rw<16>::LDS));
         BSP_HIP(allow_lds(sbr_rows_kernel<16, true>, Rw<16>::LDS));
-        BSP_HIP(allow_lds(sbr_rows_kernel<8, false>, Rw<8>::LDS));
-        BSP_HIP(allow_lds(sbr_rows_kernel<8, true>, Rw<8>::LDS));
+        BSP_HIP(allow_lds(sbr_rows8_kernel<false, 0>(), Rw<8>::LDS));
+        BSP_HIP(allow_lds(sbr_rows8_kernel<true, 0>(), Rw<8>::LDS));
+        BSP_HIP(allow_lds(sbr_rows8_kernel<false, 1>(), Rw<8>::LDS));
+        BSP_HIP(allow_lds(sbr_rows8_kernel<true, 1>(), Rw<8>::LDS));
+        BSP_HIP(allow_lds(sbr_rows8_kernel<false, 2>(), Rw<8>::LDS));
+        BSP_HIP(allow_lds(sbr_rows8_kernel<true, 2>(), Rw<8>::LDS));
+        BSP_HIP(allow_lds(sbr_rows8_kernel<false, 3>(), Rw<8>::LDS));
+        BSP_HIP(allow_lds(sbr_rows8_kernel<true, 3>(), Rw<8>::LDS));
         BSP_HIP(allow_lds(sbr_rows_general_kernel<8, false>, Rw<8>::LDS));
         BSP_HIP(allow_lds(sbr_rows_general_kernel<8, true>, Rw<8>::LDS));
         int nb = 0;
@@ -1344,15 +1482,27 @@
     const int fab = opts().sb2st_force_abort;
     const bool phased = opts().sbr_phased != 0;
     const int lagmode = opts().sbr_lag;
+    const int xdpp = opts().sbr_xdpp < 0 ? 0 : (opts().sbr_xdpp > 3 ? 3 : opts().sbr_xdpp);
     auto launch = [&](long long *dbuf) {
         if (rows) hipLaunchKernelGGL(band_tail_zero_kernel, dim3(batch), dim3(256), 0, st, n, npad, 2 * hb, d_AB);
 #define SBR_LAUNCH(K, ...) hipLaunchKernelGGL((K<__VA_ARGS__>), dim3(nblk), dim3(SB16R_THREADS), Rw<8>::LDS, st, n, npad, batch, d_AB, d_d, d_e, dbuf, \
                                               d_ctl, P, d_status, fab, lagmode)
-        if (hb == 8 && dbuf && phased) SBR_LAUNCH(sbr_rows_kernel, 8, true);
-        else if (hb == 8 && dbuf) SBR_LAUNCH(sbr_rows_general_kernel, 8, true);
-        else if (hb == 8 && phased) SBR_LAUNCH(sbr_rows_kernel, 8, false);
-        else if (hb == 8) SBR_LAUNCH(sbr_rows_general_kernel, 8, false);
+#define SBR_LAUNCH8(K) hipLaunchKernelGGL(K, dim3(nblk), dim3(SB16R_THREADS), Rw<8>::LDS, st, n, npad, batch, d_AB, d_d, d_e, dbuf, d_ctl, P, d_status, \
+                                          fab, lagmode)
+        if (hb == 8 && dbuf && phased) {
+            if (xdpp == 3) SBR_LAUNCH8((sbr_rows8_kernel<true, 3>()));
+            else if (xdpp == 2) SBR_LAUNCH8((sbr_rows8_kernel<true, 2>()));
+            else if (xdpp == 1) SBR_LAUNCH8((sbr_rows8_kernel<true, 1>()));
+            else SBR_LAUNCH8((sbr_rows8_kernel<true, 0>()));
+        } else if (hb == 8 && dbuf) SBR_LAUNCH(sbr_rows_general_kernel, 8, true);
+        else if (hb == 8 && phased) {
+            if (xdpp == 3) SBR_LAUNCH8((sbr_rows8_kernel<false, 3>()));
+            else if (xdpp == 2) SBR_LAUNCH8((sbr_rows8_kernel<false, 2>()));
+            else if (xdpp == 1) SBR_LAUNCH8((sbr_rows8_kernel<false, 1>()));
+            else SBR_LAUNCH8((sbr_rows8_kernel<false, 0>()));
+        } else if (hb == 8) SBR_LAUNCH(sbr_rows_general_kernel, 8, false);
 #undef SBR_LAUNCH
+#undef SBR_LAUNCH8
         else if (rows && dbuf)
             hipLaunchKernelGGL((sbr_rows_kernel<16, true>), dim3(nblk), dim3(SB16R_THREADS), Rw<16>::LDS, st, n, npad, batch, d_AB, d_d, d_e, dbuf,
                                d_ctl, P, d_status, fab, 1);
```

Measured after the change: 2172 eigensolves/s, median of 6. 1.03x the previous value.
